# sriram-0311/MC-SLAM

Hardware: AMD Instinct MI355X
Metric: multi-cam frames/sec (4-cam 1280x720 @2000 kpts/cam, extract + intra-rig match) (higher is better)
Workload: dtype u8; 1 GPU; 4-cam rig 1280x720, 2000 kpts/cam, extract + all-pairs intra-rig match (configs[1]); slots=4, frames_per_launch=128, cameras=4, nfeatures=2000

## Files before the change

include/mcorb.h:

```cpp
#ifndef MCORB_H
#define MCORB_H

#include <stdint.h>
#include <stddef.h>

#ifdef __cplusplus
extern "C" {
#endif

#define MCORB_OK 0
#define MCORB_E_EMPTY (-1)
#define MCORB_E_SIZE (-2)
#define MCORB_E_CAP (-3)
#define MCORB_E_ARG (-4)
#define MCORB_E_HIP (-5)
#define MCORB_E_NODEVICE (-6)
#define MCORB_E_STATE (-7)
#define MCORB_E_OVERFLOW (-8)

#define MCORB_MAX_LEVELS 16
#define MCORB_MAX_CAMS 16
#define MCORB_SELECT_AUTO 0
#define MCORB_SELECT_HOST 1
#define MCORB_SELECT_GPU 2
// ... 10 lines not shown
    float scale_factor;
    int nlevels;
    int ini_th_fast;
    int min_th_fast;
    int orientation;
    int device_id;
    int host_threads;
    int cand_cap;
    int selection;
    int gpu_jobs;
    int reserved[5];
} mcorb_params;

void mcorb_default_params(mcorb_params *p);
const char *mcorb_last_error(void);
const char *mcorb_version(void);
int mcorb_device_count(void);

typedef struct mcorb_rig mcorb_rig;

int mcorb_rig_create(const mcorb_params *p, int ncams, int width, int height, int max_frames,
                     int nslots, mcorb_rig **out);
void mcorb_rig_destroy(mcorb_rig *r);

int mcorb_rig_upload_u8(mcorb_rig *r, int slot, const uint8_t *const *images, int nimg, int stride);
int mcorb_rig_staging(mcorb_rig *r, int slot, int m, uint8_t **ptr, int *stride);
int mcorb_rig_upload_staged(mcorb_rig *r, int slot, int nimg);
int mcorb_rig_upload_f32(mcorb_rig *r, int slot, const float *const *images, int nimg,
                         int stride_bytes, int channels);

int mcorb_rig_extract_submit(mcorb_rig *r, int slot, int nimg, int lap_x0, int lap_x1);
int mcorb_rig_extract_wait(mcorb_rig *r, int slot);
int mcorb_rig_extract(mcorb_rig *r, int slot, int nimg, int lap_x0, int lap_x1);

int mcorb_rig_process_submit(mcorb_rig *r, int slot, int nframes, int lap_x0, int lap_x1,
                             float dist_thresh, float ratio);
int mcorb_rig_process_wait(mcorb_rig *r, int slot);
int mcorb_rig_process(mcorb_rig *r, int slot, int nframes, int lap_x0, int lap_x1, float dist_thresh, float ratio);

int mcorb_rig_num_keypoints(mcorb_rig *r, int slot, int m);
int mcorb_rig_get_features(mcorb_rig *r, int slot, int m, mcorb_keypoint *kps, uint8_t *desc, int cap,
                           int *n_out, int *mono_index_out);

int mcorb_rig_set_undistortion(mcorb_rig *r, int cam, const double *K, const double *dist, int ncoeffs);
int mcorb_rig_undistortion_active(mcorb_rig *r, int cam);
int mcorb_rig_get_features_undist(mcorb_rig *r, int slot, int m, mcorb_keypoint *kps, int cap, int *n_out);

int mcorb_rig_set_image_undistortion(mcorb_rig *r, int cam, const double *K, const double *dist, int ncoeffs);
int mcorb_rig_image_undistortion_active(mcorb_rig *r, int cam);
int mcorb_rig_get_undistort_map(mcorb_rig *r, int cam, int16_t *map1_xy, uint16_t *map2, int cap_pixels);
int mcorb_rig_get_raw_image(mcorb_rig *r, int slot, int m, uint8_t *dst, int dst_stride);
int mcorb_host_undistort_map(const double *K, const double *dist, int ncoeffs, int w, int h, int16_t *map1_xy, uint16_t *map2);
int mcorb_host_remap_u8(const uint8_t *src, int src_stride, int w, int h, const int16_t *map1_xy, const uint16_t *map2,
                        uint8_t *dst, int dst_stride);

int mcorb_rig_match(mcorb_rig *r, int slot, int nframes, float dist_thresh, float ratio);
int mcorb_rig_match_submit(mcorb_rig *r, int slot, int nframes, float dist_thresh, float ratio);
int mcorb_rig_match_wait(mcorb_rig *r, int slot);
int mcorb_rig_get_pair_matches(mcorb_rig *r, int slot, int frame, int cam_i, int cam_j,
                               uint32_t *idx1, uint32_t *idx2, int cap, int *n_out);
int mcorb_rig_get_pair_knn2(mcorb_rig *r, int slot, int frame, int cam_i, int cam_j,
                            int32_t *idx, int32_t *dist, int cap_rows, int *nq_out);
int mcorb_rig_get_tracks(mcorb_rig *r, int slot, int frame, int32_t *tracks, int cap_tracks,
                         int *ntracks_out, int *mergeable_out);

int mcorb_rig_get_tracks_epipolar(mcorb_rig *r, int slot, int frame, const double *F, const mcorb_keypoint *const *kps_undist,
                                  int32_t *tracks, int cap_tracks, int *ntracks_out, int *mergeable_out);

int mcorb_rig_level_size(mcorb_rig *r, int level, int *w, int *h);
int mcorb_rig_get_level(mcorb_rig *r, int slot, int m, int level, uint8_t *dst, int dst_stride);
int mcorb_rig_get_blurred(mcorb_rig *r, int slot, int m, int level, uint8_t *dst, int dst_stride);
int mcorb_rig_get_candidates(mcorb_rig *r, int slot, int m, int level, uint32_t *packed, int cap, int *n_out);

int mcorb_rig_last_timing(mcorb_rig *r, int slot, float us[10]);
int mcorb_rig_select_mode(mcorb_rig *r);
int mcorb_rig_select_fallbacks(mcorb_rig *r, int slot);
int mcorb_rig_early_reads_rejected(mcorb_rig *r, int slot);
int mcorb_rig_set_graph(mcorb_rig *r, int every);
int mcorb_dev_sort_selftest(int device, const uint32_t *keys, int n, uint32_t *perm_dev, uint32_t *perm_std);

int mcorb_rig_kcap(mcorb_rig *r);
int mcorb_rig_host_threads(mcorb_rig *r);
int mcorb_rig_info(mcorb_rig *r, int32_t out[8]);
void *mcorb_rig_desc_device_ptr(mcorb_rig *r, int slot);
void *mcorb_rig_stream(mcorb_rig *r, int slot);
int mcorb_rig_export_descriptors(mcorb_rig *r, int slot, void *dst_dev, int32_t *counts_host, int nimg);
int mcorb_rig_match_external(mcorb_rig *r, int slot, const void *desc_dev, const int32_t *counts, int ntotal,
                             const int32_t *sets, int nframes, float dist_thresh, float ratio);
int mcorb_rig_match_external_submit(mcorb_rig *r, int slot, const void *desc_dev, const int32_t *counts, int ntotal,
                                    const int32_t *sets, int nframes, float dist_thresh, float ratio);

int mcorb_rig_export_descriptors_dev(mcorb_rig *r, int slot, void *dst_dev, int32_t *counts_dev, int nimg, void *then_stream);
int mcorb_rig_match_external_dev_submit(mcorb_rig *r, int slot, const void *desc_dev, const int32_t *counts_dev, int ntotal,
                                        const int32_t *sets, int nframes, float dist_thresh, float ratio, void *after_stream);

int mcorb_rig_match_pairs_external(mcorb_rig *r, int slot, const void *desc_dev, const int32_t *counts, int ntotal,
                                   const int32_t *pair_sets, int npairs, float dist_thresh, float ratio);
int mcorb_rig_match_pairs_external_dev_submit(mcorb_rig *r, int slot, const void *desc_dev, const int32_t *counts_dev, int ntotal,
                                              const int32_t *pair_sets, int npairs, float dist_thresh, float ratio, void *after_stream);
int mcorb_rig_get_pairlist(mcorb_rig *r, int slot, int pair, uint32_t *idx1, uint32_t *idx2, int cap, int *n_out);
int mcorb_host_merge_tracks(int ncams, const int32_t *counts, const uint32_t *const *idx1, const uint32_t *const *idx2,
                            const int32_t *npair, int32_t *tracks, int cap_tracks, int *ntracks_out, int *mergeable_out);

typedef struct mcorb_descblock mcorb_descblock;
int mcorb_descblock_create(int device, int nsets, int kcap, mcorb_descblock **out);
void mcorb_descblock_destroy(mcorb_descblock *b);
int mcorb_descblock_upload(mcorb_descblock *b, int set, const uint8_t *desc, int n);
void *mcorb_descblock_desc_ptr(mcorb_descblock *b);
int32_t *mcorb_descblock_counts_dev(mcorb_descblock *b);
int mcorb_rig_match_sets(mcorb_rig *r, int slot, mcorb_descblock *b, const int32_t *pair_sets, int npairs, float dist_thresh, float ratio);
int mcorb_rig_get_pairknn2(mcorb_rig *r, int slot, int pair, int32_t *idx, int32_t *dist, int cap_rows, int *nq_out);

typedef struct mcorb_extractor mcorb_t;

int mcorb_create(const mcorb_params *p, int max_width, int max_height, mcorb_t **out);
void mcorb_destroy(mcorb_t *e);
int mcorb_extract(mcorb_t *e, const uint8_t *gray, int w, int h, int stride_bytes,
                  int lap_x0, int lap_x1, mcorb_keypoint *kps, uint8_t *desc, int cap,
                  int *n_out, int *mono_index_out);
int mcorb_extract_f32(mcorb_t *e, const float *img01, int w, int h, int stride_bytes, int channels,
                      int lap_x0, int lap_x1, mcorb_keypoint *kps, uint8_t *desc, int cap,
                      int *n_out, int *mono_index_out);
int mcorb_get_tables(const mcorb_params *p, float *scale, float *inv_scale, float *sigma2,
                     float *inv_sigma2, int *features_per_level);
int mcorb_get_pyramid_level(mcorb_t *e, int level, uint8_t *dst, int dst_stride, int *w, int *h);

int mcorb_hamming256(const uint8_t a[32], const uint8_t b[32]);
int mcorb_representative_desc(const uint8_t *descs, int n);
int mcorb_knn2(mcorb_t *e, const uint8_t *q, int nq, const uint8_t *t, int nt, int32_t *idx, int32_t *dist);
int mcorb_match_ratio(mcorb_t *e, const uint8_t *q, int nq, const uint8_t *t, int nt,
                      float dist_thresh, float ratio, uint32_t *idx1, uint32_t *idx2, int cap, int *n_out);

typedef struct mcorb_vocab mcorb_vocab;
int mcorb_vocab_create(int k, int L, int scoring, int weighting, const int32_t *parent, const uint8_t *is_leaf,
                       const uint8_t *desc, const double *weight, int nnodes, int device, mcorb_vocab **out);
int mcorb_vocab_load_text(const char *path, int device, mcorb_vocab **out);
void mcorb_vocab_destroy(mcorb_vocab *v);
int mcorb_vocab_info(const mcorb_vocab *v, int *k, int *L, int *nnodes, int *nwords);
int mcorb_vocab_transform(mcorb_vocab *v, const uint8_t *desc, int n, int levelsup, uint32_t *bow_ids, double *bow_vals,
                          int bow_cap, int *nbow, uint32_t *fv_nodes, int32_t *fv_offsets, int fv_cap, int *nfv,
                          int32_t *fv_feats, int feat_cap);
int mcorb_rig_transform_image(mcorb_rig *r, int slot, int m, mcorb_vocab *v, int levelsup, uint32_t *bow_ids,
                              double *bow_vals, int bow_cap, int *nbow, uint32_t *fv_nodes, int32_t *fv_offsets,
                              int fv_cap, int *nfv, int32_t *fv_feats, int feat_cap);

int mcorb_rig_transform_images(mcorb_rig *r, int slot, int img0, int nimg, mcorb_vocab *v, int levelsup);
int mcorb_rig_get_transform(mcorb_rig *r, int slot, int m, uint32_t *bow_ids, double *bow_vals, int bow_cap, int *nbow,
                            uint32_t *fv_nodes, int32_t *fv_offsets, int fv_cap, int *nfv, int32_t *fv_feats, int feat_cap);
int mcorb_rig_match_bow(mcorb_rig *r, int slot, int frame, mcorb_vocab *v, int levelsup, double max_neighbor_ratio,
                        int32_t *tracks, int32_t *n_rays, int cap_tracks, int *ntracks_out, uint32_t *words,
                        int cap_words, int *nwords_out);
int mcorb_rig_match_bow_frames(mcorb_rig *r, int slot, int frame0, int nframes, mcorb_vocab *v, int levelsup,
                               double max_neighbor_ratio, const float *const *y_undist);
int mcorb_rig_get_bow_tracks(mcorb_rig *r, int slot, int frame, int32_t *tracks, int32_t *n_rays, int cap_tracks,
                             int *ntracks_out, uint32_t *words, int cap_words, int *nwords_out);

#define MCORB_BOW_TRANSFORM 1
#define MCORB_BOW_MATCH 2
#define MCORB_BOW_MAX_KCAP 4096
int mcorb_rig_set_vocabulary(mcorb_rig *r, mcorb_vocab *v, int levelsup, double max_neighbor_ratio, int flags);

typedef struct mcorb_camera {
    double K[9];
    double Rt[12];
} mcorb_camera;
typedef struct mcorb_lf_feature {
// ... 188 lines not shown
    int32_t *match_dist;
    double *match_pt;
    int32_t n_proj[MCORB_MAX_CAMS], n_match[MCORB_MAX_CAMS];
    int32_t n_candidates, reserved;
} mcorb_track_out;
int mcorb_lmap_track(mcorb_lmap *m, const mcorb_track_view *view, const mcorb_track_frame *frame, const int32_t *lids, int n_lids,
                     double max_d2, int max_hamming, mcorb_track_out *out);
int mcorb_lmap_track_rig_frame(mcorb_lmap *m, const mcorb_track_view *view, mcorb_rig *r, int slot, int frame, const int32_t *lids,
                               int n_lids, double max_d2, int max_hamming, mcorb_track_out *out);
int mcorb_lmap_last_track_timing(mcorb_lmap *m, float us[2]);
int mcorb_lmap_last_track_timing4(mcorb_lmap *m, float us[4]);
int mcorb_lmap_last_track_timing5(mcorb_lmap *m, float us[5]);
int mcorb_lmap_track_submit(mcorb_lmap *m, const mcorb_track_view *view, const mcorb_track_frame *frame, const int32_t *lids, int n_lids,
                            double max_d2, int max_hamming, int want_pts);
int mcorb_lmap_track_rig_frame_submit(mcorb_lmap *m, const mcorb_track_view *view, mcorb_rig *r, int slot, int frame, const int32_t *lids,
                                      int n_lids, double max_d2, int max_hamming, int want_pts);
int mcorb_lmap_track_wait(mcorb_lmap *m, mcorb_track_out *out);
#define MCORB_TRACK_MAX_FRAMES 32
int mcorb_lmap_track_rig_frames_submit(mcorb_lmap *m, const mcorb_track_view *views, mcorb_rig *r, int slot, const int32_t *frames, int nf,
                                       const int32_t *lids, const int32_t *lid_first , double max_d2, int max_hamming,
                                       int want_pts);
int mcorb_lmap_track_frames_wait(mcorb_lmap *m, mcorb_track_out *outs, int n_outs);
int mcorb_lmap_track_rig_frames(mcorb_lmap *m, const mcorb_track_view *views, mcorb_rig *r, int slot, const int32_t *frames, int nf,
                                const int32_t *lids, const int32_t *lid_first, double max_d2, int max_hamming, int want_pts,
                                mcorb_track_out *outs);

#define MCORB_POSE_LANES 256
#define MCORB_POSE_NO_OBS 0
#define MCORB_POSE_NO_STEP 1
#define MCORB_POSE_CONVERGED 2
#define MCORB_POSE_MAX_ITER 3
typedef struct mcorb_pose_params {
    double inv_sigma2[MCORB_MAX_LEVELS];
    int32_t nlevels, max_iterations;
} mcorb_pose_params;
typedef struct mcorb_pose_result {
    double R[9], t[3];
    double cost_initial, cost_final;
    int32_t status, iterations[2], n_inliers, n_obs, reserved;
} mcorb_pose_result;
int mcorb_lmap_refine_pose(mcorb_lmap *m, int n, const int32_t *cam, const float *uv, const int32_t *octave, const int32_t *lids,
                           const double *pts, int ncams, const mcorb_track_cam *cams, const double *R, const double *t,
                           const mcorb_pose_params *params, mcorb_pose_result *res, uint8_t *inlier);
int mcorb_lmap_last_pose_timing(mcorb_lmap *m, float us[1]);
int mcorb_lmap_set_track_refine(mcorb_lmap *m, const mcorb_pose_params *params);
int mcorb_lmap_last_track_pose(mcorb_lmap *m, int f, mcorb_pose_result *out, uint8_t *flags, int cap);
void mcorb_pose_of_view(const mcorb_track_view *view, double R[9], double t[3]);
int mcorb_pose_eval(int ncams, const mcorb_track_cam *cams, int n, const int32_t *cam, const float *uv, const double *pts, const double *R,
                    const double *t, double *r, double *J, double *w);

#define MCORB_SAC_MAX_ITERATIONS 1024
#define MCORB_SAC_SOLVER_CENTRAL 0
#define MCORB_SAC_SOLVER_RIG 1
#define MCORB_SAC_OK 0
#define MCORB_SAC_NO_OBS 1
#define MCORB_SAC_NO_MODEL 2
typedef struct mcorb_sac_params {
    double threshold;
    uint64_t seed;
    int32_t max_iterations, solver;
} mcorb_sac_params;
typedef struct mcorb_sac_result {
    double R[9], t[3];
    double sac_R[9], sac_t[3];
    int32_t status, used, n_inliers, n_matches;
    int32_t sac_n_inliers, best_hypothesis, sample[4], n_models, n_consensus;
    mcorb_pose_result refine;
} mcorb_sac_result;
int mcorb_lmap_ransac_pose(mcorb_lmap *m, int n, const int32_t *cam, const float *uv, const int32_t *octave, const int32_t *match,
                           const int32_t *lids, const double *pts, int ncams, const mcorb_track_cam *cams,
                           const mcorb_sac_params *params, const mcorb_pose_params *refine_params, mcorb_sac_result *res,
                           uint8_t *inlier);
int mcorb_lmap_last_ransac_timing(mcorb_lmap *m, float us[3], int *n_hyp);
int mcorb_lmap_last_ransac_counts(mcorb_lmap *m, int32_t *count, int32_t *valid, int cap, int *n_hyp);
double mcorb_sac_threshold(double K00_02);
int mcorb_sac_solve(const mcorb_track_cam *cam, const float *uv, const double *pts, double *R, double *t);
int mcorb_sac_solve_rig(int ncams, const mcorb_track_cam *cams, const int32_t *cam, const float *uv, const double *pts, double *R, double *t);
int mcorb_sac_eval(int ncams, const mcorb_track_cam *cams, int n, const int32_t *cam, const float *uv, const double *pts, const double *R,
                   const double *t, double *score);

int mcorb_host_select(const uint32_t *packed, int n, int minX, int maxX, int minY, int maxY,
                      int nfeatures_level, int wCell, int hCell, int32_t *out_idx, int cap);
int mcorb_host_resize_axis(int ssize, int dsize, int is_x, int32_t *quads);
int mcorb_host_geometry(const mcorb_params *p, int w, int h, int32_t *six_per_level);
int mcorb_host_triangulate(const double *x, const double *P, int nv, double X[3]);
int mcorb_host_triangulate_branch(const double *x, const double *P, int nv, double X[3], int32_t *branch);
int32_t mcorb_host_track_pixel(float v);

int mcorb_synth_rig_frame(uint32_t frame, int ncams, int cam, int w, int h, uint8_t *out, int stride);

#ifdef __cplusplus
}
#endif
#endif
```

mc-slam_amd/__init__.py:

```python
import ctypes as C

import numpy as np

from . import _lib
from ._lib import (E_ARG, E_CAP, E_EMPTY, E_HIP, E_NODEVICE, E_OVERFLOW, E_SIZE, E_STATE, KP_DTYPE, OBS_RECORD, OBS_UPDATE, OK,
                   ORIENT_IC_ANGLE, ORIENT_NONE, McorbError, Params, default_params)
from .synth import synth_rig_frame, synth_rig_frame_numpy

TH_HIGH = 100
TH_LOW = 75
HISTO_LENGTH = 30


def _u8(a):
    return np.ascontiguousarray(a, dtype=np.uint8)


def device_count():
    return _lib.load().mcorb_device_count()


def get_tables(params):
    n = params.nlevels
    sc, isc, s2, is2 = (np.zeros(n, np.float32) for _ in range(4))
    q = np.zeros(n, np.int32)
    _lib.check(_lib.load().mcorb_get_tables(C.byref(params), sc.ctypes.data, isc.ctypes.data, s2.ctypes.data,
                                            is2.ctypes.data, q.ctypes.data))
    return dict(scale=sc, inv_scale=isc, sigma2=s2, inv_sigma2=is2, quota=q)


def hamming256(a, b):
    a, b = _u8(a).reshape(32), _u8(b).reshape(32)
    return _lib.load().mcorb_hamming256(a.ctypes.data, b.ctypes.data)


def representative_desc(descs):
    d = _u8(descs).reshape(-1, 32)
    r = _lib.load().mcorb_representative_desc(d.ctypes.data, len(d))
    if r < 0:
        _lib.check(r)
    return r


class Rig:

    def __init__(self, ncams, width, height, max_frames=1, nslots=1, params=None, **kw):
        self.L = _lib.load()
        self.params = params if params is not None else default_params(**kw)
        self.ncams, self.w, self.h, self.max_frames, self.nslots = ncams, width, height, max_frames, nslots
        h = C.c_void_p()
        _lib.check(self.L.mcorb_rig_create(C.byref(self.params), ncams, width, height, max_frames, nslots, C.byref(h)))
        self.h_rig = h
        self.kcap = self.L.mcorb_rig_kcap(h)
        self.nlevels = self.params.nlevels

    def close(self):
        if getattr(self, "h_rig", None):
            self.L.mcorb_rig_destroy(self.h_rig)
            self.h_rig = None

    def __del__(self):
        try:
            self.close()
        except Exception:
            pass

    def upload(self, images, slot=0):
        first = np.asarray(images[0])
        if first.dtype == np.uint8:
            arrs = [_u8(im) for im in images]
            for a in arrs:
                if a.shape != (self.h, self.w):
                    raise ValueError("image shape %s != (%d,%d)" % (a.shape, self.h, self.w))
            ptrs = (C.c_void_p * len(arrs))(*[a.ctypes.data for a in arrs])
            _lib.check(self.L.mcorb_rig_upload_u8(self.h_rig, slot, ptrs, len(arrs), self.w))
        else:
            arrs = [np.ascontiguousarray(im, dtype=np.float32) for im in images]
            ch = 1 if arrs[0].ndim == 2 else arrs[0].shape[2]
            ptrs = (C.c_void_p * len(arrs))(*[a.ctypes.data for a in arrs])
            _lib.check(self.L.mcorb_rig_upload_f32(self.h_rig, slot, ptrs, len(arrs), arrs[0].strides[0], ch))
        return len(arrs)

    def staging(self, m, slot=0):
        ptr, stride = C.c_void_p(), C.c_int()
        _lib.check(self.L.mcorb_rig_staging(self.h_rig, slot, m, C.byref(ptr), C.byref(stride)))
        buf = (C.c_uint8 * (self.h * stride.value)).from_address(ptr.value)
        return np.frombuffer(buf, np.uint8).reshape(self.h, stride.value)[:, :self.w]

    def upload_staged(self, nimg, slot=0):
        _lib.check(self.L.mcorb_rig_upload_staged(self.h_rig, slot, nimg))

    def extract(self, nimg, slot=0, lap=(0, 0)):
        _lib.check(self.L.mcorb_rig_extract(self.h_rig, slot, nimg, lap[0], lap[1]))

# ... 176 lines not shown
            for c in range(Cn):
                a = np.ascontiguousarray(kps_undist[c], _lib.KP_DTYPE)
                keep.append(a)
                undp[c] = a.ctypes.data
        wp = None
        if words is not None:
            words = np.ascontiguousarray(words, np.uint32)
            assert len(words) >= len(tracks)
            wp = words.ctypes.data
        cap = max(total_feats, len(tracks)) + 1
        out = np.empty(cap, _lib.LF_DTYPE)
        wf = np.zeros(len(tracks) + 1, np.uint32)
        n, ni, nm, nw = (C.c_int() for _ in range(4))
        _lib.check(self.L.mcorb_rig_obtain_lf_features(self.h_rig, slot, frame, tracks.ctypes.data, len(tracks), wp, cams, segp, stride, undp,
                                                       total_feats, out.ctypes.data, cap, C.byref(n), C.byref(ni), C.byref(nm),
                                                       wf.ctypes.data, len(wf), C.byref(nw)))
        return out[:n.value].copy(), ni.value, nm.value, wf[:nw.value].copy()

    def obtain_lf_features_frames(self, frame0, tracks_per_frame, K_mats, R_mats, t_mats, words_per_frame=None, seg_masks=None,
                                  kps_undist=None, total_feats=3000, slot=0):
        Cn, F = self.ncams, len(tracks_per_frame)
        trs = [np.ascontiguousarray(t, np.int32).reshape(-1, Cn) for t in tracks_per_frame]
        nt = np.array([len(t) for t in trs], np.int32)
        tracks = np.ascontiguousarray(np.concatenate(trs) if nt.sum() else np.zeros((0, Cn), np.int32))
        cams = (_lib.Camera * Cn)()
        for c in range(Cn):
            K = np.asarray(K_mats[c], np.float64).reshape(3, 3)
            Rt = np.hstack([np.asarray(R_mats[c], np.float64).reshape(3, 3), np.asarray(t_mats[c], np.float64).reshape(3, 1)])
            cams[c].K[:] = K.ravel().tolist()
            cams[c].Rt[:] = Rt.ravel().tolist()
        keep, segp, stride = [], None, 0
        if seg_masks is not None:
            segp = (C.c_void_p * (F * Cn))()
            for i in range(F * Cn):
                if seg_masks[i] is not None:
                    a = np.ascontiguousarray(seg_masks[i], np.float32)
                    assert stride in (0, a.shape[1]), "all segmentation masks must share one row stride"
                    keep.append(a)
                    segp[i] = a.ctypes.data
                    stride = a.shape[1]
        undp = None
        if kps_undist is not None:
            undp = (C.c_void_p * (F * Cn))()
            for i in range(F * Cn):
                a = np.ascontiguousarray(kps_undist[i], _lib.KP_DTYPE)
                keep.append(a)
                undp[i] = a.ctypes.data
        wp = None
        if words_per_frame is not None:
            ws = [np.ascontiguousarray(w, np.uint32)[:n] for w, n in zip(words_per_frame, nt)]
            assert all(len(w) == n for w, n in zip(ws, nt)), "one word per track"
            words = np.ascontiguousarray(np.concatenate(ws) if nt.sum() else np.zeros(0, np.uint32))
            keep.append(words)
            wp = words.ctypes.data
        cap = max(total_feats, int(nt.max(initial=0))) + 1
        capw = int(nt.max(initial=0)) + 1
        out = np.empty((F, cap), _lib.LF_DTYPE)
        wf = np.zeros((F, capw), np.uint32)
        n, ni, nm, nw = (np.zeros(F, np.int32) for _ in range(4))
        _lib.check(self.L.mcorb_rig_obtain_lf_features_frames(self.h_rig, slot, frame0, F, tracks.ctypes.data, nt.ctypes.data, wp, cams, segp,
                                                              stride, undp, total_feats, out.ctypes.data, cap, n.ctypes.data, ni.ctypes.data,
                                                              nm.ctypes.data, wf.ctypes.data, capw, nw.ctypes.data))
        return [(out[f, :n[f]].copy(), int(ni[f]), int(nm[f]), wf[f, :nw[f]].copy()) for f in range(F)]

    def level_size(self, level):
        w, h = C.c_int(), C.c_int()
        _lib.check(self.L.mcorb_rig_level_size(self.h_rig, level, C.byref(w), C.byref(h)))
        return w.value, h.value

    def level(self, m, level, slot=0, blurred=False):
        w, h = self.level_size(level)
        out = np.zeros((h, w), np.uint8)
        fn = self.L.mcorb_rig_get_blurred if blurred else self.L.mcorb_rig_get_level
        _lib.check(fn(self.h_rig, slot, m, level, out.ctypes.data, w))
        return out

    def candidates(self, m, level, slot=0, cap=1 << 17):
        buf = np.zeros(cap, np.uint32)
        n = C.c_int()
        _lib.check(self.L.mcorb_rig_get_candidates(self.h_rig, slot, m, level, buf.ctypes.data, cap, C.byref(n)))
        p = buf[:n.value]
        return ((p >> 8) & 0xfff).astype(np.int32), (p >> 20).astype(np.int32), (p & 0xff).astype(np.int32)

    def info(self):
        o = np.zeros(8, np.int32)
        _lib.check(self.L.mcorb_rig_info(self.h_rig, o.ctypes.data))
        d = dict(zip(("kcap", "cells", "tiles", "cell_cap", "cand_cap", "bucket_total", "img_bytes", "nlevels"), (int(v) for v in o)))
        d["host_threads"] = int(self.L.mcorb_rig_host_threads(self.h_rig))
        return d

    def select_mode(self):
        return {1: "host", 2: "gpu"}[self.L.mcorb_rig_select_mode(self.h_rig)]

    def set_graph(self, every):
        _lib.check(self.L.mcorb_rig_set_graph(self.h_rig, every))

    def select_fallbacks(self, slot=0):
        return int(self.L.mcorb_rig_select_fallbacks(self.h_rig, slot))

    def early_reads_rejected(self, slot=0):
        return int(self.L.mcorb_rig_early_reads_rejected(self.h_rig, slot))

    def timing(self, slot=0):
        t = (C.c_float * 10)()
        _lib.check(self.L.mcorb_rig_last_timing(self.h_rig, slot, t))
        return dict(phase_a_us=t[0], select_us=t[1], phase_b_us=t[2], match_us=t[3], pyramid_us=t[4],
                    fast_us=t[5], compact_us=t[6], knn2_us=t[7], blur_us=t[8], describe_us=t[9])

    def export_descriptors(self, dst_dev_ptr, nimg, slot=0):
        counts = np.zeros(nimg, np.int32)
        _lib.check(self.L.mcorb_rig_export_descriptors(self.h_rig, slot, dst_dev_ptr, counts.ctypes.data, nimg))
        return counts

    def match_external(self, desc_dev_ptr, counts, sets, slot=0, dist_thresh=75.0, ratio=0.85):
        self.match_external_submit(desc_dev_ptr, counts, sets, slot, dist_thresh, ratio)
        self.match_wait(slot)

    def match_external_submit(self, desc_dev_ptr, counts, sets, slot=0, dist_thresh=75.0, ratio=0.85):
        counts = np.ascontiguousarray(counts, np.int32)
        sets = np.ascontiguousarray(sets, np.int32).reshape(-1, self.ncams)
        self._keep = getattr(self, "_keep", {})
        self._keep[slot] = (counts, sets)
        _lib.check(self.L.mcorb_rig_match_external_submit(self.h_rig, slot, desc_dev_ptr, counts.ctypes.data, len(counts),
                                                          sets.ctypes.data, len(sets), dist_thresh, ratio))

    def export_descriptors_dev(self, dst_dev_ptr, counts_dev_ptr, nimg, slot=0, then_stream=None):
        if then_stream:
            _lib.require_torch_first("export_descriptors_dev")
        _lib.check(self.L.mcorb_rig_export_descriptors_dev(self.h_rig, slot, dst_dev_ptr, counts_dev_ptr, nimg, then_stream))

    def match_external_dev_submit(self, desc_dev_ptr, counts_dev_ptr, ntotal, sets, slot=0, dist_thresh=75.0, ratio=0.85,
                                  after_stream=None):
        if after_stream:
            _lib.require_torch_first("match_external_dev_submit")
        sets = np.ascontiguousarray(sets, np.int32).reshape(-1, self.ncams)
        self._keep = getattr(self, "_keep", {})
        self._keep[slot] = (sets,)
        _lib.check(self.L.mcorb_rig_match_external_dev_submit(self.h_rig, slot, desc_dev_ptr, counts_dev_ptr, int(ntotal),
                                                              sets.ctypes.data, len(sets), dist_thresh, ratio, after_stream))

    def match_wait(self, slot=0):
        _lib.check(self.L.mcorb_rig_match_wait(self.h_rig, slot))

    def match_pairs_external(self, desc_dev_ptr, counts, pair_sets, slot=0, dist_thresh=75.0, ratio=0.85):
        counts = np.ascontiguousarray(counts, np.int32)
        pair_sets = np.ascontiguousarray(pair_sets, np.int32).reshape(-1, 2)
        _lib.check(self.L.mcorb_rig_match_pairs_external(self.h_rig, slot, desc_dev_ptr, counts.ctypes.data, len(counts),
                                                         pair_sets.ctypes.data, len(pair_sets), dist_thresh, ratio))

    def match_pairs_external_dev_submit(self, desc_dev_ptr, counts_dev_ptr, ntotal, pair_sets, slot=0, dist_thresh=75.0, ratio=0.85,
                                        after_stream=None):
        if after_stream:
            _lib.require_torch_first("match_pairs_external_dev_submit")
        pair_sets = np.ascontiguousarray(pair_sets, np.int32).reshape(-1, 2)
        self._keep = getattr(self, "_keep", {})
        self._keep[slot] = (pair_sets,)
        _lib.check(self.L.mcorb_rig_match_pairs_external_dev_submit(self.h_rig, slot, desc_dev_ptr, counts_dev_ptr, int(ntotal),
                                                                    pair_sets.ctypes.data, len(pair_sets), dist_thresh, ratio, after_stream))

    def match_sets(self, block, pair_sets, slot=0, dist_thresh=75.0, ratio=0.85):
        pair_sets = np.ascontiguousarray(pair_sets, np.int32).reshape(-1, 2)
        _lib.check(self.L.mcorb_rig_match_sets(self.h_rig, slot, block.h, pair_sets.ctypes.data, len(pair_sets), dist_thresh, ratio))

    def pairknn2(self, pair, slot=0):
        idx, dist = np.zeros((self.kcap, 2), np.int32), np.zeros((self.kcap, 2), np.int32)
        n = C.c_int()
        _lib.check(self.L.mcorb_rig_get_pairknn2(self.h_rig, slot, pair, idx.ctypes.data, dist.ctypes.data, self.kcap, C.byref(n)))
        return idx[:n.value].copy(), dist[:n.value].copy()

    def pairlist(self, pair, slot=0):
        i1, i2 = np.zeros(self.kcap, np.uint32), np.zeros(self.kcap, np.uint32)
        n = C.c_int()
# ... 1309 lines not shown
```

mc-slam_amd/_lib.py:

```python
import ctypes as C
import os
import sys

import numpy as np

PKG_DIR = os.path.dirname(os.path.abspath(__file__))
LIB_PATH = os.path.join(PKG_DIR, "libmcorb.so")

OK, E_EMPTY, E_SIZE, E_CAP, E_ARG, E_HIP, E_NODEVICE, E_STATE, E_OVERFLOW = 0, -1, -2, -3, -4, -5, -6, -7, -8
ORIENT_NONE, ORIENT_IC_ANGLE = 0, 1
BOW_TRANSFORM, BOW_MATCH = 1, 2
OBS_UPDATE, OBS_RECORD = 0, 1
MAX_LEVELS, MAX_CAMS = 16, 16
TRACK_KNN, TRACK_TILE = 10, 1024
TRACK_MAX_FRAMES = 32
POSE_LANES = 256
POSE_NO_OBS, POSE_NO_STEP, POSE_CONVERGED, POSE_MAX_ITER = 0, 1, 2, 3

KP_DTYPE = np.dtype([("x", "<f4"), ("y", "<f4"), ("size", "<f4"), ("angle", "<f4"),
                     ("response", "<f4"), ("octave", "<i4"), ("class_id", "<i4")])


class Params(C.Structure):
    _fields_ = [("nfeatures", C.c_int), ("scale_factor", C.c_float), ("nlevels", C.c_int),
# ... 76 lines not shown
    _fields_ = [("R", C.c_double * 9), ("t", C.c_double * 3), ("cost_initial", C.c_double), ("cost_final", C.c_double),
                ("status", C.c_int32), ("iterations", C.c_int32 * 2), ("n_inliers", C.c_int32), ("n_obs", C.c_int32),
                ("reserved", C.c_int32)]


class SacParams(C.Structure):
    _fields_ = [("threshold", C.c_double), ("seed", C.c_uint64), ("max_iterations", C.c_int32), ("solver", C.c_int32)]


class SacResultC(C.Structure):
    _fields_ = [("R", C.c_double * 9), ("t", C.c_double * 3), ("sac_R", C.c_double * 9), ("sac_t", C.c_double * 3),
                ("status", C.c_int32), ("used", C.c_int32), ("n_inliers", C.c_int32), ("n_matches", C.c_int32),
                ("sac_n_inliers", C.c_int32), ("best_hypothesis", C.c_int32), ("sample", C.c_int32 * 4), ("n_models", C.c_int32),
                ("n_consensus", C.c_int32), ("refine", PoseResultC)]


class McorbError(RuntimeError):
    def __init__(self, code, msg):
        super().__init__("mcorb error %d: %s" % (code, msg))
        self.code = code


_vp, _i, _f = C.c_void_p, C.c_int, C.c_float
_ip = C.POINTER(C.c_int)

SIGNATURES = {
    "mcorb_default_params": (None, [C.POINTER(Params)]),
    "mcorb_last_error": (C.c_char_p, []),
    "mcorb_version": (C.c_char_p, []),
    "mcorb_device_count": (_i, []),
    "mcorb_rig_create": (_i, [C.POINTER(Params), _i, _i, _i, _i, _i, C.POINTER(_vp)]),
    "mcorb_rig_destroy": (None, [_vp]),
    "mcorb_rig_upload_u8": (_i, [_vp, _i, C.POINTER(_vp), _i, _i]),
    "mcorb_rig_upload_f32": (_i, [_vp, _i, C.POINTER(_vp), _i, _i, _i]),
    "mcorb_rig_extract_submit": (_i, [_vp, _i, _i, _i, _i]),
    "mcorb_rig_extract_wait": (_i, [_vp, _i]),
    "mcorb_rig_extract": (_i, [_vp, _i, _i, _i, _i]),
    "mcorb_rig_staging": (_i, [_vp, _i, _i, _vp, _ip]),
    "mcorb_rig_upload_staged": (_i, [_vp, _i, _i]),
    "mcorb_rig_process_submit": (_i, [_vp, _i, _i, _i, _i, _f, _f]),
    "mcorb_rig_process": (_i, [_vp, _i, _i, _i, _i, _f, _f]),
    "mcorb_rig_process_wait": (_i, [_vp, _i]),
    "mcorb_rig_num_keypoints": (_i, [_vp, _i, _i]),
    "mcorb_rig_get_features": (_i, [_vp, _i, _i, _vp, _vp, _i, _ip, _ip]),
    "mcorb_rig_set_undistortion": (_i, [_vp, _i, _vp, _vp, _i]),
    "mcorb_rig_undistortion_active": (_i, [_vp, _i]),
    "mcorb_rig_get_features_undist": (_i, [_vp, _i, _i, _vp, _i, _ip]),
    "mcorb_rig_set_image_undistortion": (_i, [_vp, _i, _vp, _vp, _i]),
    "mcorb_rig_image_undistortion_active": (_i, [_vp, _i]),
    "mcorb_rig_get_undistort_map": (_i, [_vp, _i, _vp, _vp, _i]),
    "mcorb_rig_get_raw_image": (_i, [_vp, _i, _i, _vp, _i]),
    "mcorb_host_undistort_map": (_i, [_vp, _vp, _i, _i, _i, _vp, _vp]),
    "mcorb_host_remap_u8": (_i, [_vp, _i, _i, _i, _vp, _vp, _vp, _i]),
    "mcorb_rig_match": (_i, [_vp, _i, _i, _f, _f]),
    "mcorb_rig_match_submit": (_i, [_vp, _i, _i, _f, _f]),
    "mcorb_rig_match_wait": (_i, [_vp, _i]),
    "mcorb_rig_get_pair_matches": (_i, [_vp, _i, _i, _i, _i, _vp, _vp, _i, _ip]),
    "mcorb_rig_get_pair_knn2": (_i, [_vp, _i, _i, _i, _i, _vp, _vp, _i, _ip]),
    "mcorb_rig_get_tracks": (_i, [_vp, _i, _i, _vp, _i, _ip, _ip]),
    "mcorb_rig_level_size": (_i, [_vp, _i, _ip, _ip]),
    "mcorb_rig_get_level": (_i, [_vp, _i, _i, _i, _vp, _i]),
    "mcorb_rig_get_blurred": (_i, [_vp, _i, _i, _i, _vp, _i]),
    "mcorb_rig_get_candidates": (_i, [_vp, _i, _i, _i, _vp, _i, _ip]),
    "mcorb_rig_last_timing": (_i, [_vp, _i, C.POINTER(_f)]),
    "mcorb_rig_select_mode": (_i, [_vp]),
    "mcorb_rig_select_fallbacks": (_i, [_vp, _i]),
    "mcorb_rig_early_reads_rejected": (_i, [_vp, _i]),
    "mcorb_rig_set_graph": (_i, [_vp, _i]),
    "mcorb_dev_sort_selftest": (_i, [_i, _vp, _i, _vp, _vp]),
    "mcorb_rig_match_pairs_external": (_i, [_vp, _i, _vp, _vp, _i, _vp, _i, _f, _f]),
    "mcorb_rig_match_pairs_external_dev_submit": (_i, [_vp, _i, _vp, _vp, _i, _vp, _i, _f, _f, _vp]),
    "mcorb_rig_get_pairlist": (_i, [_vp, _i, _i, _vp, _vp, _i, _ip]),
    "mcorb_host_merge_tracks": (_i, [_i, _vp, _vp, _vp, _vp, _vp, _i, _ip, _ip]),
    "mcorb_descblock_create": (_i, [_i, _i, _i, _vp]),
    "mcorb_descblock_destroy": (None, [_vp]),
    "mcorb_descblock_upload": (_i, [_vp, _i, _vp, _i]),
    "mcorb_descblock_desc_ptr": (_vp, [_vp]),
    "mcorb_descblock_counts_dev": (_vp, [_vp]),
    "mcorb_rig_match_sets": (_i, [_vp, _i, _vp, _vp, _i, _f, _f]),
    "mcorb_rig_get_pairknn2": (_i, [_vp, _i, _i, _vp, _vp, _i, _ip]),
    "mcorb_rig_kcap": (_i, [_vp]),
    "mcorb_rig_host_threads": (_i, [_vp]),
    "mcorb_rig_info": (_i, [_vp, _vp]),
    "mcorb_rig_desc_device_ptr": (_vp, [_vp, _i]),
    "mcorb_rig_stream": (_vp, [_vp, _i]),
    "mcorb_rig_export_descriptors": (_i, [_vp, _i, _vp, _vp, _i]),
    "mcorb_rig_match_external": (_i, [_vp, _i, _vp, _vp, _i, _vp, _i, _f, _f]),
    "mcorb_rig_match_external_submit": (_i, [_vp, _i, _vp, _vp, _i, _vp, _i, _f, _f]),
    "mcorb_rig_export_descriptors_dev": (_i, [_vp, _i, _vp, _vp, _i, _vp]),
    "mcorb_rig_match_external_dev_submit": (_i, [_vp, _i, _vp, _vp, _i, _vp, _i, _f, _f, _vp]),
    "mcorb_create": (_i, [C.POINTER(Params), _i, _i, C.POINTER(_vp)]),
    "mcorb_destroy": (None, [_vp]),
    "mcorb_extract": (_i, [_vp, _vp, _i, _i, _i, _i, _i, _vp, _vp, _i, _ip, _ip]),
    "mcorb_extract_f32": (_i, [_vp, _vp, _i, _i, _i, _i, _i, _i, _vp, _vp, _i, _ip, _ip]),
    "mcorb_get_tables": (_i, [C.POINTER(Params), _vp, _vp, _vp, _vp, _vp]),
    "mcorb_get_pyramid_level": (_i, [_vp, _i, _vp, _i, _ip, _ip]),
    "mcorb_hamming256": (_i, [_vp, _vp]),
    "mcorb_representative_desc": (_i, [_vp, _i]),
    "mcorb_knn2": (_i, [_vp, _vp, _i, _vp, _i, _vp, _vp]),
    "mcorb_match_ratio": (_i, [_vp, _vp, _i, _vp, _i, _f, _f, _vp, _vp, _i, _ip]),
    "mcorb_vocab_create": (_i, [_i, _i, _i, _i, _vp, _vp, _vp, _vp, _i, _i, C.POINTER(_vp)]),
    "mcorb_vocab_load_text": (_i, [C.c_char_p, _i, C.POINTER(_vp)]),
    "mcorb_vocab_destroy": (None, [_vp]),
    "mcorb_vocab_info": (_i, [_vp, _ip, _ip, _ip, _ip]),
    "mcorb_vocab_transform": (_i, [_vp, _vp, _i, _i, _vp, _vp, _i, _ip, _vp, _vp, _i, _ip, _vp, _i]),
    "mcorb_rig_transform_image": (_i, [_vp, _i, _i, _vp, _i, _vp, _vp, _i, _ip, _vp, _vp, _i, _ip, _vp, _i]),
    "mcorb_rig_get_tracks_epipolar": (_i, [_vp, _i, _i, _vp, _vp, _vp, _i, _ip, _ip]),
    "mcorb_rig_match_bow": (_i, [_vp, _i, _i, _vp, _i, C.c_double, _vp, _vp, _i, _ip, _vp, _i, _ip]),
    "mcorb_rig_transform_images": (_i, [_vp, _i, _i, _i, _vp, _i]),
    "mcorb_rig_get_transform": (_i, [_vp, _i, _i, _vp, _vp, _i, _ip, _vp, _vp, _i, _ip, _vp, _i]),
    "mcorb_rig_match_bow_frames": (_i, [_vp, _i, _i, _i, _vp, _i, C.c_double, _vp]),
    "mcorb_rig_set_vocabulary": (_i, [_vp, _vp, _i, C.c_double, _i]),
    "mcorb_rig_get_bow_tracks": (_i, [_vp, _i, _i, _vp, _vp, _i, _ip, _vp, _i, _ip]),
    "mcorb_rig_obtain_lf_features": (_i, [_vp, _i, _i, _vp, _i, _vp, _vp, _vp, _i, _vp, _i, _vp, _i, _ip, _ip, _ip, _vp, _i, _ip]),
    "mcorb_rig_obtain_lf_features_frames": (_i, [_vp, _i, _i, _i, _vp, _vp, _vp, _vp, _vp, _i, _vp, _i, _vp, _i, _vp, _vp, _vp, _vp, _i, _vp]),
    "mcorb_host_select": (_i, [_vp, _i, _i, _i, _i, _i, _i, _i, _i, _vp, _i]),
    "mcorb_host_resize_axis": (_i, [_i, _i, _i, _vp]),
    "mcorb_host_triangulate": (_i, [_vp, _vp, _i, _vp]),
    "mcorb_host_triangulate_branch": (_i, [_vp, _vp, _i, _vp, _vp]),
    "mcorb_rig_set_lf": (_i, [_vp, _vp, _i]),
    "mcorb_rig_get_lf_features": (_i, [_vp, _i, _i, _vp, _i, _ip, _ip, _ip, _vp, _i, _ip]),
    "mcorb_rig_get_lf_bow": (_i, [_vp, _i, _i, _vp, _vp, _i, _ip, _vp, _vp, _i, _ip, _vp, _i]),
    "mcorb_dev_triangulate_selftest": (_i, [_i, _vp, _vp, _vp, _i, _vp, _vp]),
    "mcorb_kfdb_create": (_i, [_vp, _i, _i, _i, _i, C.POINTER(_vp)]),
    "mcorb_kfdb_destroy": (None, [_vp]),
    "mcorb_kfdb_add": (_i, [_vp, _vp, _vp, _i, _vp, _vp, _i, _vp, _vp, _i, _ip]),
    "mcorb_kfdb_add_rig_frame": (_i, [_vp, _vp, _i, _i, _ip]),
    "mcorb_kfdb_size": (_i, [_vp]),
    "mcorb_kfdb_get_entry": (_i, [_vp, _i, _vp, _vp, _i, _ip, _vp, _vp, _i, _ip, _vp, _i, _vp, _i, _ip]),
    "mcorb_kfdb_query": (_i, [_vp, _vp, _vp, _i, _i, _i, _vp, _vp, _i, _ip]),
    "mcorb_kfdb_query_entries": (_i, [_vp, _vp, _vp, _i, _i, _vp, _vp, _i, _vp]),
    "mcorb_kfdb_score": (_i, [_vp, _i, _i, C.POINTER(C.c_double)]),
    "mcorb_kfdb_feature_matches": (_i, [_vp, _i, _i, C.c_double, _vp, _vp, _i, _ip]),
    "mcorb_kfdb_last_timing": (_i, [_vp, C.POINTER(_f)]),
    "mcorb_kfdb_reserve_probes": (_i, [_vp, _i]),
    "mcorb_kfdb_set_probe": (_i, [_vp, _i, _vp, _vp, _i, _vp, _vp, _i, _vp, _vp, _i]),
    "mcorb_kfdb_set_probe_rig_frame": (_i, [_vp, _i, _vp, _i, _i]),
    "mcorb_kfdb_get_probe": (_i, [_vp, _i, _vp, _vp, _i, _ip, _vp, _vp, _i, _ip, _vp, _i, _vp, _i, _ip]),
    "mcorb_kfdb_query_probes": (_i, [_vp, _vp, _vp, _i, _i, _vp, _vp, _i, _vp]),
    "mcorb_kfdb_score_probe": (_i, [_vp, _i, _i, C.POINTER(C.c_double)]),
    "mcorb_kfdb_probe_feature_matches": (_i, [_vp, _i, _vp, _i, C.c_double, _vp, _vp, _i, _vp]),
    "mcorb_kfdb_probe_inter_matches_bf": (_i, [_vp, _i, _i, _vp, _vp, _vp, _vp, _vp, _vp, _vp, _vp, _i, _ip]),
    "mcorb_kfdb_last_probe_timing": (_i, [_vp, C.POINTER(_f)]),
    "mcorb_lmap_create": (_i, [_vp, _i, _i, _i, C.POINTER(_vp)]),
    "mcorb_lmap_destroy": (None, [_vp]),
    "mcorb_lmap_set": (_i, [_vp, _vp, _i, _vp, _vp, _vp, _vp]),
    "mcorb_lmap_set_desc_from_entry": (_i, [_vp, _vp, _i, _vp, _vp, _i, _vp]),
    "mcorb_lmap_get": (_i, [_vp, _i, _vp, _vp, _vp, _ip, _ip]),
    "mcorb_lmap_search": (_i, [_vp, C.POINTER(LmapView), _vp, _i, _vp, _i, _vp, _i, _vp, _vp, _vp, _i, C.c_double, _vp, _vp, _i, _ip,
                               _vp, _vp, _i, _ip, _vp, _vp, _i, _ip]),
    "mcorb_lmap_last_timing": (_i, [_vp, C.POINTER(_f), _ip]),
    "mcorb_lmap_triangulate_neighbours": (_i, [_vp, C.POINTER(MapFrame), _vp, C.POINTER(MapFrame), C.POINTER(_vp), _i, C.POINTER(_vp),
                                               C.POINTER(_vp), C.POINTER(_vp), _vp, _vp, _vp, _i, _vp, _vp, C.c_int32,
                                               C.POINTER(MapOut)]),
    "mcorb_lmap_depths": (_i, [_vp, _vp, _vp, _vp, _i, _vp]),
    "mcorb_lmap_last_triangulate_timing": (_i, [_vp, C.POINTER(_f), _ip, _ip]),
    "mcorb_lmap_triangulate_new": (_i, [_vp, C.POINTER(MapFrame), _vp, C.POINTER(MapFrame), _vp, _vp, _vp, _i, _vp, _vp, _i, _i,
                                        C.POINTER(MapNewOut)]),
    "mcorb_lmap_last_triangulate_new_timing": (_i, [_vp, C.POINTER(_f), _ip]),
    "mcorb_host_map_refine": (_i, [_i] + [_vp] * 11 + [_i] + [_vp] * 5),
    "mcorb_dev_map_refine_selftest": (_i, [_i, _i] + [_vp] * 11 + [_i] + [_vp] * 5),
    "mcorb_host_map_gates": (_i, [_i, _vp, _vp, _vp, _vp, _vp, _vp, _vp, _vp, _vp, _vp, _i, _vp, _vp, _vp]),
    "mcorb_dev_map_gates_selftest": (_i, [_i, _i, _vp, _vp, _vp, _vp, _vp, _vp, _vp, _vp, _vp, _vp, _i, _vp, _vp, _vp]),
    "mcorb_lmap_set_rays": (_i, [_vp, _vp, _i, _vp]),
    "mcorb_lmap_get_observations": (_i, [_vp, _i, C.POINTER(C.c_int32), _vp, _vp, _i, _ip]),
    "mcorb_lmap_observe": (_i, [_vp, C.POINTER(ObsFrame), _vp, _vp, _i, _i, _vp, _i, _vp, _vp]),
    "mcorb_lmap_update_points": (_i, [_vp, _vp, _i, _vp, C.c_double, _vp, _vp]),
    "mcorb_lmap_delete": (_i, [_vp, _vp, _i, _vp, _vp, _i, _ip]),
    "mcorb_lmap_observers": (_i, [_vp, _vp, _i, _vp, _i, _ip]),
    "mcorb_lmap_last_landmark_timing": (_i, [_vp, C.POINTER(_f)]),
    "mcorb_lmap_track": (_i, [_vp, C.POINTER(TrackView), C.POINTER(TrackFrame), _vp, _i, C.c_double, _i, C.POINTER(TrackOut)]),
    "mcorb_lmap_track_rig_frame": (_i, [_vp, C.POINTER(TrackView), _vp, _i, _i, _vp, _i, C.c_double, _i, C.POINTER(TrackOut)]),
    "mcorb_lmap_last_track_timing": (_i, [_vp, C.POINTER(_f)]),
    "mcorb_lmap_last_track_timing4": (_i, [_vp, C.POINTER(_f)]),
    "mcorb_lmap_last_track_timing5": (_i, [_vp, C.POINTER(_f)]),
    "mcorb_lmap_track_submit": (_i, [_vp, C.POINTER(TrackView), C.POINTER(TrackFrame), _vp, _i, C.c_double, _i, _i]),
    "mcorb_lmap_track_rig_frame_submit": (_i, [_vp, C.POINTER(TrackView), _vp, _i, _i, _vp, _i, C.c_double, _i, _i]),
    "mcorb_lmap_track_wait": (_i, [_vp, C.POINTER(TrackOut)]),
    "mcorb_lmap_track_rig_frames_submit": (_i, [_vp, C.POINTER(TrackView), _vp, _i, _vp, _i, _vp, _vp, C.c_double, _i, _i]),
    "mcorb_lmap_track_frames_wait": (_i, [_vp, C.POINTER(TrackOut), _i]),
    "mcorb_lmap_track_rig_frames": (_i, [_vp, C.POINTER(TrackView), _vp, _i, _vp, _i, _vp, _vp, C.c_double, _i, _i, C.POINTER(TrackOut)]),
    "mcorb_host_track_pixel": (C.c_int32, [_f]),
    "mcorb_lmap_refine_pose": (_i, [_vp, _i, _vp, _vp, _vp, _vp, _vp, _i, _vp, _vp, _vp, C.POINTER(PoseParams), C.POINTER(PoseResultC), _vp]),
    "mcorb_lmap_last_pose_timing": (_i, [_vp, C.POINTER(_f)]),
    "mcorb_lmap_set_track_refine": (_i, [_vp, C.POINTER(PoseParams)]),
    "mcorb_lmap_last_track_pose": (_i, [_vp, _i, C.POINTER(PoseResultC), _vp, _i]),
    "mcorb_pose_of_view": (None, [C.POINTER(TrackView), _vp, _vp]),
    "mcorb_pose_eval": (_i, [_i, _vp, _i, _vp, _vp, _vp, _vp, _vp, _vp, _vp, _vp]),
    "mcorb_lmap_ransac_pose": (_i, [_vp, _i, _vp, _vp, _vp, _vp, _vp, _vp, _i, _vp, C.POINTER(SacParams), C.POINTER(PoseParams),
                                    C.POINTER(SacResultC), _vp]),
    "mcorb_lmap_last_ransac_timing": (_i, [_vp, C.POINTER(_f), C.POINTER(_i)]),
    "mcorb_lmap_last_ransac_counts": (_i, [_vp, _vp, _vp, _i, C.POINTER(_i)]),
    "mcorb_sac_threshold": (C.c_double, [C.c_double]),
    "mcorb_sac_solve": (_i, [_vp, _vp, _vp, _vp, _vp]),
    "mcorb_sac_solve_rig": (_i, [_i, _vp, _vp, _vp, _vp, _vp, _vp]),
    "mcorb_sac_eval": (_i, [_i, _vp, _i, _vp, _vp, _vp, _vp, _vp, _vp]),
    "mcorb_host_geometry": (_i, [C.POINTER(Params), _i, _i, _vp]),
    "mcorb_synth_rig_frame": (_i, [C.c_uint32, _i, _i, _i, _i, _vp, _i]),
}

# ... 41 lines not shown
```

mc-slam_amd/csrc/mcorb_api.cpp:

```cpp
#include <string.h>

#include <algorithm>
#include <cmath>
#include <chrono>
#include <new>

#include "mcorb_engine.h"

using namespace mcorb;

extern "C" {

void mcorb_default_params(mcorb_params *p)
{
    if (!p) return;
    memset(p, 0, sizeof(*p));
    p->nfeatures = 2000;
    p->scale_factor = 1.2f;
    p->nlevels = 8;
    p->ini_th_fast = 20;
    p->min_th_fast = 7;
    p->orientation = MCORB_ORIENT_NONE;
}

// ... 369 lines not shown
    Slot *s = get_slot(r, slot);
    if (!s) return MCORB_E_STATE;
    const Geom &g = r->rig.geom;
    if (m < 0 || m >= s->nimg_done || level < 0 || level >= g.nlevels) { set_error("bad candidate request"); return MCORB_E_ARG; }
    int dev_lo[kMaxLevels + 1];
    const int *lo = s->tbl(m) + kTblLvlOff;
    if (!(s->host_results && !r->rig.gpu_select)) {
        HIPCHK(hipSetDevice(r->rig.device));
        HIPCHK(hipMemcpy(dev_lo, s->d_tbl + (size_t)m * s->tbl_ints_per_image + kTblLvlOff, sizeof(dev_lo), hipMemcpyDeviceToHost));
        lo = dev_lo;
    }
    const int n = lo[level + 1] - lo[level];
    if (n_out) *n_out = n;
    if (n > cap) { set_error("candidate buffer too small"); return MCORB_E_CAP; }
    if (n) {
        std::vector<uint32_t> tmp(n);
        HIPCHK(hipSetDevice(r->rig.device));
        HIPCHK(hipMemcpy(tmp.data(), s->d_sorted + (size_t)m * g.candCap + lo[level], (size_t)n * 4, hipMemcpyDeviceToHost));
        const uint32_t *src = tmp.data();
        const int wc = g.lv[level].wCell, hc = g.lv[level].hCell;
        std::vector<std::pair<uint64_t, uint32_t>> v(n);
        for (int i = 0; i < n; i++) {
            const int x = cand_x(src[i]), y = cand_y(src[i]);
            v[i] = {((((uint64_t)((y - 3) / hc) << 12 | (uint64_t)((x - 3) / wc)) << 12 | (uint64_t)y) << 12) | (uint64_t)x, src[i]};
        }
        std::sort(v.begin(), v.end());
        for (int i = 0; i < n; i++) packed[i] = v[i].second;
    }
    return MCORB_OK;
}

int mcorb_rig_last_timing(mcorb_rig *r, int slot, float us[10])
{
    Slot *s = get_slot(r, slot);
    if (!s) return MCORB_E_STATE;
    for (int i = 0; i < T_COUNT; i++) us[i] = s->timing[i];
    return MCORB_OK;
}

int mcorb_rig_kcap(mcorb_rig *r) { return r ? r->rig.geom.kcap : MCORB_E_ARG; }
int mcorb_rig_select_mode(mcorb_rig *r) { return r ? (r->rig.gpu_select ? MCORB_SELECT_GPU : MCORB_SELECT_HOST) : MCORB_E_ARG; }
int mcorb_rig_set_graph(mcorb_rig *r, int every)
{
    if (!r || every < 0) return MCORB_E_ARG;
    r->rig.graph_every.store(r->rig.gpu_select ? every : 0);
    return MCORB_OK;
}
int mcorb_rig_select_fallbacks(mcorb_rig *r, int slot)
{
    if (!r || slot < 0 || slot >= (int)r->rig.slots.size()) return MCORB_E_ARG;
    return r->rig.slots[slot]->fallbacks.load(std::memory_order_relaxed);
}
int mcorb_rig_early_reads_rejected(mcorb_rig *r, int slot)
{
    if (!r || slot < 0 || slot >= (int)r->rig.slots.size()) return MCORB_E_ARG;
    return r->rig.slots[slot]->stale_reads.load(std::memory_order_relaxed);
}
int mcorb_dev_sort_selftest(int device, const uint32_t *keys, int n, uint32_t *dev_perm, uint32_t *std_perm)
{
    if (n < 0 || n > 6000 || (n && (!keys || !dev_perm || !std_perm))) { set_error("sort_selftest: bad argument"); return MCORB_E_ARG; }
    if (n == 0) return MCORB_OK;
    std::vector<uint64_t> a((size_t)n), b((size_t)n);
    for (int i = 0; i < n; i++) a[i] = ((uint64_t)keys[i] << 32) | (uint32_t)i;
    b = a;
    std::sort(b.begin(), b.end(), [](uint64_t x, uint64_t y) { return (x >> 32) < (y >> 32); });
    for (int i = 0; i < n; i++) std_perm[i] = (uint32_t)b[i];
    HIPCHK(hipSetDevice(device));
    DevBuf<uint64_t> d_in, d_out;
    TRY(d_in.alloc((size_t)n));
    TRY(d_out.alloc((size_t)n));
    HIPCHK(hipMemcpy(d_in, a.data(), (size_t)n * 8, hipMemcpyHostToDevice));
    HIPCHK(sort_selftest(d_in, n, d_out));
    HIPCHK(hipMemcpy(b.data(), d_out, (size_t)n * 8, hipMemcpyDeviceToHost));
    for (int i = 0; i < n; i++) dev_perm[i] = (uint32_t)b[i];
    return MCORB_OK;
}
int mcorb_rig_host_threads(mcorb_rig *r) { return r ? r->rig.pool_threads : MCORB_E_ARG; }
int mcorb_rig_info(mcorb_rig *r, int32_t out[8])
{
    if (!r || !out) return MCORB_E_ARG;
    const Geom &g = r->rig.geom;
    out[0] = g.kcap; out[1] = g.cells; out[2] = g.tiles; out[3] = g.cellCap; out[4] = g.candCap; out[5] = g.bucketTotal;
    out[6] = (int32_t)g.imgBytes; out[7] = g.nlevels;
    return MCORB_OK;
}
void *mcorb_rig_desc_device_ptr(mcorb_rig *r, int slot)
{
    if (!r || slot < 0 || slot >= (int)r->rig.slots.size()) return nullptr;
    return r->rig.slots[slot]->d_desc;
}
void *mcorb_rig_stream(mcorb_rig *r, int slot)
{
    if (!r || slot < 0 || slot >= (int)r->rig.slots.size()) return nullptr;
    return (void *)r->rig.slots[slot]->st;
}

int mcorb_rig_match_external_submit(mcorb_rig *r, int slot, const void *desc_dev, const int32_t *counts, int ntotal,
                                    const int32_t *sets, int nframes, float dist_thresh, float ratio)
{
    if (!r || !desc_dev || !counts || !sets) { set_error("null argument"); return MCORB_E_ARG; }
    Job j = match_job(nframes, dist_thresh, ratio);
    j.ext_desc = desc_dev; j.ext_counts = counts; j.ext_total = ntotal; j.ext_sets = sets;
    return r->rig.submit(slot, j);
}

int mcorb_rig_match_external(mcorb_rig *r, int slot, const void *desc_dev, const int32_t *counts, int ntotal,
                             const int32_t *sets, int nframes, float dist_thresh, float ratio)
{
    const int st = mcorb_rig_match_external_submit(r, slot, desc_dev, counts, ntotal, sets, nframes, dist_thresh, ratio);
    return st != MCORB_OK ? st : r->rig.wait(slot);
}

int mcorb_rig_match_external_dev_submit(mcorb_rig *r, int slot, const void *desc_dev, const int32_t *counts_dev, int ntotal,
                                        const int32_t *sets, int nframes, float dist_thresh, float ratio, void *after_stream)
{
    if (!r || !desc_dev || !counts_dev || !sets) { set_error("null argument"); return MCORB_E_ARG; }
    Job j = match_job(nframes, dist_thresh, ratio);
    j.ext_desc = desc_dev; j.ext_counts_dev = counts_dev; j.ext_total = ntotal; j.ext_sets = sets;
    j.after_stream = (hipStream_t)after_stream;
    if (after_stream) {
        Slot *s = get_slot(r, slot);
        if (!s) return MCORB_E_STATE;
        HIPCHK(hipSetDevice(r->rig.device));
        HIPCHK(hipEventRecord(s->ev_x, (hipStream_t)after_stream));
    }
    return r->rig.submit(slot, j);
}

int mcorb_rig_match_pairs_external_dev_submit(mcorb_rig *r, int slot, const void *desc_dev, const int32_t *counts_dev, int ntotal,
                                              const int32_t *pair_sets, int npairs, float dist_thresh, float ratio, void *after_stream)
{
    if (!r || !desc_dev || !counts_dev || !pair_sets) { set_error("null argument"); return MCORB_E_ARG; }
    Job j = match_job(0, dist_thresh, ratio);
    j.ext_desc = desc_dev; j.ext_counts_dev = counts_dev; j.ext_total = ntotal; j.ext_pairs = pair_sets; j.ext_npairs = npairs;
    j.after_stream = (hipStream_t)after_stream;
    if (after_stream) {
        Slot *s = get_slot(r, slot);
        if (!s) return MCORB_E_STATE;
        HIPCHK(hipSetDevice(r->rig.device));
        HIPCHK(hipEventRecord(s->ev_x, (hipStream_t)after_stream));
    }
    return r->rig.submit(slot, j);
}

int mcorb_rig_match_pairs_external(mcorb_rig *r, int slot, const void *desc_dev, const int32_t *counts, int ntotal,
                                   const int32_t *pair_sets, int npairs, float dist_thresh, float ratio)
{
    if (!r || !desc_dev || !counts || !pair_sets) { set_error("null argument"); return MCORB_E_ARG; }
    Job j = match_job(0, dist_thresh, ratio);
    j.ext_desc = desc_dev; j.ext_counts = counts; j.ext_total = ntotal; j.ext_pairs = pair_sets; j.ext_npairs = npairs;
    return r->rig.run_sync(slot, j);
}

int mcorb_rig_get_pairlist(mcorb_rig *r, int slot, int pair, uint32_t *idx1, uint32_t *idx2, int cap, int *n_out)
{
    if (n_out) *n_out = 0;
    Slot *s = get_slot(r, slot);
    if (!s) return MCORB_E_STATE;
    if (pair < 0 || pair >= s->npairs_done) { set_error("bad pair index"); return MCORB_E_ARG; }
    const int n = (int)s->m_idx1[pair].size();
    if (n_out) *n_out = n;
    if (n > cap || (n && (!idx1 || !idx2))) { set_error("pair list: output too small"); return MCORB_E_CAP; }
    if (n) {
        memcpy(idx1, s->m_idx1[pair].data(), (size_t)n * sizeof(uint32_t));
        memcpy(idx2, s->m_idx2[pair].data(), (size_t)n * sizeof(uint32_t));
    }
// ... 130 lines not shown
```

mc-slam_amd/csrc/mcorb_api_extractor.cpp:

```cpp
#include <string.h>

#include <algorithm>
#include <new>

#include "mcorb_engine.h"

using namespace mcorb;

struct mcorb_extractor {
    mcorb_params params;
    std::unique_ptr<Rig> rig;
    int w = 0, h = 0;
    DevBuf<uint8_t> d_desc, d_exp;
    DevBuf<int> d_lcounts;
    DevBuf<uint2> d_part;
    HostBuf<KnnRow> h_rows;
    HostBuf<uint32_t> h_mlist;
    HostBuf<int> h_mcount, h_counts;
    HostBuf<int2> h_pair;
    int kc = 0;
};

extern "C" {

// ... 166 lines not shown
        TRY(e->d_lcounts.alloc(2));
        TRY(e->h_rows.alloc((size_t)need, hipHostMallocMapped));
        TRY(e->h_mlist.alloc(knn_mlist_stride(need), hipHostMallocMapped));
        TRY(e->h_mcount.alloc((size_t)knn_qblocks(need), hipHostMallocMapped));
        TRY(e->h_counts.alloc(2, hipHostMallocMapped));
        TRY(e->h_pair.alloc(1, hipHostMallocMapped));
        e->kc = need;
    }
    if (nq) HIPCHK(hipMemcpy(e->d_desc, q, (size_t)nq * 32, hipMemcpyHostToDevice));
    if (nt) HIPCHK(hipMemcpy(e->d_desc + (size_t)e->kc * 32, t, (size_t)nt * 32, hipMemcpyHostToDevice));
    e->h_counts[0] = nq;
    e->h_counts[1] = nt;
    e->h_pair[0] = int2{0, 1};
    launch_knn2(nullptr, e->d_desc, e->h_counts, nullptr, 2, e->h_pair, 1, e->kc, e->d_exp, e->d_lcounts, e->d_part, thr, ratio, e->h_rows,
                e->h_mlist, e->h_mcount, nullptr, nullptr);
    HIPCHK(hipGetLastError());
    HIPCHK(hipStreamSynchronize(nullptr));
    return MCORB_OK;
}

int mcorb_knn2(mcorb_t *e, const uint8_t *q, int nq, const uint8_t *t, int nt, int32_t *idx, int32_t *dist)
{
    if (!idx || !dist) { set_error("null output"); return MCORB_E_ARG; }
    const int st = knn2_host_arrays(e, q, nq, t, nt, 75.f, 0.85f);
    if (st != MCORB_OK) return st;
    decode_rows(e->h_rows, nq, idx, dist);
    return MCORB_OK;
}

int mcorb_match_ratio(mcorb_t *e, const uint8_t *q, int nq, const uint8_t *t, int nt, float dist_thresh, float ratio,
                      uint32_t *idx1, uint32_t *idx2, int cap, int *n_out)
{
    const int st = knn2_host_arrays(e, q, nq, t, nt, dist_thresh, ratio);
    if (st != MCORB_OK) return st;
    int n = 0;
    for (int i = 0; i < nq; i++) {
        const KnnRow &r = e->h_rows[i];
        if (knn_accept(r)) {
            if (n < cap) { idx1[n] = (uint32_t)i; idx2[n] = (uint32_t)knn_idx0(r); }
            n++;
        }
    }
    if (n_out) *n_out = n;
    if (n > cap) { set_error("match buffer too small"); return MCORB_E_CAP; }
    return MCORB_OK;
}

int mcorb_host_select(const uint32_t *packed, int n, int minX, int maxX, int minY, int maxY, int nfeatures_level,
                      int wCell, int hCell, int32_t *out_idx, int cap)
{
    if (n < 0 || (n && !packed) || !out_idx) { set_error("host_select: bad argument"); return MCORB_E_ARG; }
    if (n == 0) return 0;
    const SelectParams P = make_select_params(minX, maxX, minY, maxY, nfeatures_level, wCell, hCell);
    if (P.nIni < 1) { set_error("host_select: level too tall"); return MCORB_E_SIZE; }
    static thread_local SelectScratch sc;
    std::vector<uint32_t> sorted;
    std::vector<int> perm, bstart;
    std::vector<mcorb::BucketBest> bbest;
    host_bucket_sort(packed, n, P, sorted, perm, bstart, bbest);
    std::vector<int> out((size_t)std::max(nfeatures_level, 0) + 64 + 8);
    std::vector<uint32_t> outv(out.size());
    const int r = select_octree(sorted.data(), bstart.data(), bbest.data(), n, P, out.data(), outv.data(), sc);
    if (r == -4) { set_error("host_select: 2^20 candidates or a level 4096 px wide: beyond the packed (count, UL.x) sort key"); return MCORB_E_SIZE; }
    if (r < 0) { set_error("host_select: level too tall"); return MCORB_E_SIZE; }
    if (r > cap) { set_error("host_select: output too small"); return MCORB_E_CAP; }
    for (int i = 0; i < r; i++) {
        out_idx[i] = perm[out[i]];
        if (outv[i] != packed[out_idx[i]]) { set_error("host_select: value/index mismatch"); return MCORB_E_STATE; }
    }
    return r;
}

int mcorb_host_resize_axis(int ssize, int dsize, int is_x, int32_t *quads)
{
    if (ssize < 1 || dsize < 1 || !quads) return MCORB_E_ARG;
    std::vector<ResizeTap> t;
    build_resize_axis(ssize, dsize, is_x != 0, t, 1);
    for (int d = 0; d < dsize; d++) {
        quads[4 * d] = t[d].s0; quads[4 * d + 1] = t[d].s1; quads[4 * d + 2] = t[d].c0; quads[4 * d + 3] = t[d].c1;
    }
    return MCORB_OK;
}

int mcorb_host_geometry(const mcorb_params *p, int w, int h, int32_t *six)
{
    if (!p || !six) return MCORB_E_ARG;
    Tables t;
    int st = compute_tables(*p, t);
    if (st != MCORB_OK) return st;
    Geom g;
    std::vector<ResizeTap> taps;
    st = build_geometry(*p, t, w, h, g, taps);
    if (st != MCORB_OK) return st;
    for (int l = 0; l < g.nlevels; l++) {
        const LevelGeom &L = g.lv[l];
        int32_t *o = six + 6 * l;
        o[0] = L.w; o[1] = L.h; o[2] = L.nCols; o[3] = L.nRows; o[4] = L.wCell; o[5] = L.hCell;
    }
    return MCORB_OK;
}

}
```

mc-slam_amd/csrc/mcorb_common.h:

```cpp
#pragma once
#include <stdint.h>
#include <stddef.h>

namespace mcorb {

constexpr int kMaxLevels = 16;
constexpr int kEdge = 19;
constexpr int kMinBorder = 16;
constexpr int kCellW = 35;
constexpr int kMaxRoi = 76;
constexpr int kResizeTileH = 32;
constexpr int kBlurTW = 128, kBlurTH = 32;
constexpr int kTilePitch = 80;

__host__ __device__ inline uint32_t pack_cand(int x, int y, int resp) { return ((uint32_t)y << 20) | ((uint32_t)x << 8) | (uint32_t)resp; }
__host__ __device__ inline int cand_x(uint32_t p) { return (int)((p >> 8) & 0xfffu); }
__host__ __device__ inline int cand_y(uint32_t p) { return (int)(p >> 20); }
__host__ __device__ inline int cand_resp(uint32_t p) { return (int)(p & 0xffu); }

constexpr int kPickOrderMask = (1 << 23) - 1;
struct BucketBest { uint32_t key, pos, val; };
struct BucketWin { uint32_t key, val; };

constexpr int kTblLvlOff = 0, kTblShipped = kMaxLevels + 1, kTblHead = 48;
// ... 34 lines not shown
__host__ __device__ inline void unpack_sel(uint32_t v, int &level, int &x, int &y)
{
    level = (int)(v >> 28);
    y = (int)((v >> 14) & 0x3fffu);
    x = (int)(v & 0x3fffu);
}

constexpr int kBlurTileRows = 8, kBlurTileCols = 16, kBlurTileBytes = 128;
#if defined(__HIPCC__)
__host__ __device__
#endif
inline size_t blur_tiled_offset(int pitch, int x, int y)
{
    return ((size_t)(y >> 3) * (size_t)(pitch >> 4) + (size_t)(x >> 4)) * kBlurTileBytes + (size_t)((y & 7) << 4) + (size_t)(x & 15);
}

struct LevelGeom {
    int w, h;
    int pitch;
    uint32_t off;
    int nCols, nRows;
    int wCell, hCell;
    int cell0;
    int tile0;
    int tilesX, tilesY;
    int maxBorderX, maxBorderY;
    uint32_t xtab, ytab;
    int nIni;
    float hX;
    int depth;
    int nBuckets;
    int bucket0;
    int quota;
    uint32_t lutx, luty;
};

struct Geom {
    int nlevels;
    int cells;
    int tiles;
    int cellCap;
    uint32_t imgBytes;
    int kcap;
    int candCap;
    int hostCandCap;
    int bucketTotal;
    LevelGeom lv[kMaxLevels];
};

__host__ __device__ inline uint32_t path_code(int x, int y, int W0, int H0, int nIni, float hX, int depth)
{
#if defined(__HIP_DEVICE_COMPILE__)
    int r = (int)__fdiv_rn((float)x, hX);
    if (r >= nIni) r = nIni - 1;
    int x0 = (int)__fmul_rn(hX, (float)r), x1 = (int)__fmul_rn(hX, (float)(r + 1));
#else
    int r = (int)((float)x / hX);
    if (r >= nIni) r = nIni - 1;
    int x0 = (int)(hX * (float)r), x1 = (int)(hX * (float)(r + 1));
#endif
    int y0 = 0, y1 = H0;
    (void)W0;
    uint32_t code = (uint32_t)r;
    for (int d = 0; d < depth; d++) {
        const int sx = x0 + ((x1 - x0 + 1) >> 1), sy = y0 + ((y1 - y0 + 1) >> 1);
        const int qx = x >= sx, qy = y >= sy;
        if (qx) x0 = sx; else x1 = sx;
        if (qy) y0 = sy; else y1 = sy;
        code = (code << 2) | (uint32_t)(qx + 2 * qy);
    }
    return code;
}

inline void path_code_tables(int W0, int H0, int nIni, float hX, int depth, uint16_t *tx, uint16_t *ty)
{
    uint32_t ymask = 0;
    for (int d = 0; d < depth; d++) ymask |= 2u << (2 * d);
    for (int x = 0; x < W0; x++) tx[x] = (uint16_t)(path_code(x, 0, W0, H0, nIni, hX, depth) & ~ymask);
    for (int y = 0; y < H0; y++) ty[y] = (uint16_t)(path_code(0, y, W0, H0, nIni, hX, depth) & ymask);
}

struct ResizeTap { uint16_t s0, s1; int16_t c0, c1; };

}
```

mc-slam_amd/csrc/mcorb_engine.cpp:

```cpp
#include <stdlib.h>
#include <string.h>
#include <sys/prctl.h>
#include <time.h>

#include "mcorb_engine.h"
#include "mcorb_prof.h"

namespace mcorb {

static thread_local std::string g_err;
void set_error(const std::string &msg) { g_err = msg; }
const char *get_error() { return g_err.c_str(); }
hipError_t Rig::wait_event(hipEvent_t ev) const
{
    if (wait_mode != 2) return hipEventSynchronize(ev);
    for (int i = 0;; i++) {
        const hipError_t e = hipEventQuery(ev);
        if (e != hipErrorNotReady) return e;
        if (i < 4) { std::this_thread::yield(); continue; }
        timespec ts = {0, 20000};
        nanosleep(&ts, nullptr);
    }
}

template <typename T>
static int host_alloc(HostBuf<T> &b, size_t n)
{
    TRY(b.alloc(n, kHostMapped));
    memset(b, 0, n * sizeof(T));
    return MCORB_OK;
}

int Rig::init(const mcorb_params &p, int ncams_, int W_, int H_, int max_frames_, int nslots)
{
    if (ncams_ < 1 || ncams_ > MCORB_MAX_CAMS || max_frames_ < 1 || nslots < 1 || W_ < 1 || H_ < 1) {
        set_error("bad rig arguments");
        return MCORB_E_ARG;
    }
    int ndev = 0;
    if (hipGetDeviceCount(&ndev) != hipSuccess || ndev <= 0 || p.device_id < 0 || p.device_id >= ndev) {
        set_error("no usable HIP device (libmcorb has no CPU path)");
        return MCORB_E_NODEVICE;
    }
    hipDeviceProp_t prop;
    HIPCHK(hipGetDeviceProperties(&prop, p.device_id));
    if (strncmp(prop.gcnArchName, "gfx950", 6) != 0) {
        set_error(std::string("device is ") + prop.gcnArchName + ", libmcorb is built for gfx950 only");
        return MCORB_E_NODEVICE;
    }
    params = p;
    ncams = ncams_; W = W_; H = H_; max_frames = max_frames_;
    max_images = ncams * max_frames;
    undist_cams.assign(ncams, UndistCam{});
    undist_set.assign(ncams, 0);
    imgud_cams.assign(ncams, UndistImageCam{});
    imgud_set.assign(ncams, 0);
    imgud_map1.assign(ncams, {});
    imgud_map2.assign(ncams, {});
    d_imgud_map1.resize(ncams);
    d_imgud_map2.resize(ncams);
    npp = ncams * (ncams - 1) / 2;
    device = p.device_id;
    HIPCHK(hipSetDevice(device));
    TRY(compute_tables(p, tab));
    std::vector<ResizeTap> taps;
    std::vector<uint16_t> lut;
    TRY(build_geometry(p, tab, W, H, geom, taps, &lut));
    for (int l = 0; l < geom.nlevels; l++)
        selp[l] = make_select_params(kMinBorder, geom.lv[l].maxBorderX, kMinBorder, geom.lv[l].maxBorderY, tab.quota[l],
                                     geom.lv[l].wCell, geom.lv[l].hCell);
    if (taps.empty()) taps.push_back(ResizeTap{0, 0, 0, 0});
    TRY(resize_windows(geom, taps, resize_win));
    TRY(d_taps.alloc(taps.size()));
    HIPCHK(hipMemcpy(d_taps, taps.data(), taps.size() * sizeof(ResizeTap), hipMemcpyHostToDevice));
    TRY(d_lut.alloc(lut.size() + 8));
    HIPCHK(hipMemcpy(d_lut, lut.data(), lut.size() * sizeof(uint16_t), hipMemcpyHostToDevice));
    {
        std::vector<uint32_t> ft;
        fast_cell_off = fast_cell_table(geom, ft);
        TRY(d_fasttab.alloc(ft.size()));
        HIPCHK(hipMemcpy(d_fasttab, ft.data(), ft.size() * sizeof(uint32_t), hipMemcpyHostToDevice));
    }
    HIPCHK(upload_umax(tab.umax));

    const int cores = usable_cores();
    const char *sync_env = getenv("MCORB_SYNC");
    wait_mode = nslots > 1 ? 2 : 0;
    if (sync_env) wait_mode = !strcmp(sync_env, "block") ? 1 : (!strcmp(sync_env, "poll") ? 2 : 0);
    const bool blocking = wait_mode == 1;
    int nthreads = p.host_threads > 0 ? p.host_threads : (wait_mode == 0 ? cores - nslots - 2 : cores - 4);
    if (p.host_threads <= 0) nthreads = std::max(2, std::min(nthreads, std::min(max_images, 16)));
    if (getenv("MCORB_HOST_THREADS")) nthreads = atoi(getenv("MCORB_HOST_THREADS"));
    nthreads = std::max(1, std::min(nthreads, 64));
    blur_planes = p.orientation != 0 || getenv("MCORB_BLUR_PLANES") != nullptr;
    copy_kernel = getenv("MCORB_COPY_KERNEL") ? atoi(getenv("MCORB_COPY_KERNEL")) != 0 : nslots == 1;
    {
        const char *e = getenv("MCORB_SELECT");
        int mode = p.selection;
        if (mode == MCORB_SELECT_AUTO && e) mode = !strcmp(e, "host") ? MCORB_SELECT_HOST : (!strcmp(e, "gpu") ? MCORB_SELECT_GPU : MCORB_SELECT_AUTO);
        if (mode != MCORB_SELECT_AUTO && mode != MCORB_SELECT_HOST && mode != MCORB_SELECT_GPU) { set_error("mcorb_params.selection: unknown mode"); return MCORB_E_ARG; }
        gpu_select = mode != MCORB_SELECT_HOST && select_fits(geom);
        if (gpu_select) HIPCHK(configure_select(geom));
        if (getenv("MCORB_SELECT_DEEP_CAP")) select_deep_cap = std::max(1, atoi(getenv("MCORB_SELECT_DEEP_CAP")));
        compact_one_copy = getenv("MCORB_COMPACT_ONE_COPY") != nullptr;
        select_prof = getenv("MCORB_SELECT_PROF") != nullptr;
        gpu_job_limit = getenv("MCORB_GPU_JOBS") ? atoi(getenv("MCORB_GPU_JOBS")) : p.gpu_jobs;
        if (gpu_job_limit < 0 || gpu_job_limit >= nslots) gpu_job_limit = 0;
        upload_pipelined = !(getenv("MCORB_UPLOAD_PIPE") && atoi(getenv("MCORB_UPLOAD_PIPE")) == 0);
        graph_every = !gpu_select ? 0 : getenv("MCORB_GRAPH") ? std::max(0, atoi(getenv("MCORB_GRAPH"))) : (nslots == 1 ? 1 : 0);
    }
    pool.reset(new WorkerPool(nthreads));
    pool_threads = nthreads;
    for (int i = 0; i < nthreads + nslots; i++) scratch.emplace_back(new SelectScratch);

    const int npairs_max = std::max(1, npp * max_frames);
    ext_cap = (int)align_up(std::max((size_t)4096, (size_t)64 * max_images), 64);
    for (int si = 0; si < nslots; si++) {
        slots.emplace_back(new Slot);
        Slot *s = slots.back().get();
        s->rig = this;
        s->index = si;
        for (Stream *st : {&s->st, &s->st_copy, &s->st_dma}) TRY(st->create(hipStreamNonBlocking));
        TRY(s->ev_x.create(hipEventDisableTiming));
        for (Event *e : {&s->ev_c, &s->ev_e, &s->ev_start, &s->ev_pyr, &s->ev_fast, &s->ev_blur, &s->ev_desc0, &s->ev_desc1, &s->ev_knn0, &s->ev_knn1, &s->ev_fin})
            TRY(e->create(hipEventDefault));
        for (Event *e : {&s->ev_tables, &s->ev_done, &s->ev_side}) TRY(e->create(blocking ? hipEventBlockingSync : hipEventDefault));
        const size_t M = (size_t)max_images;
        TRY(s->d_pyr.alloc(M * geom.imgBytes));
        HIPCHK(hipMemset(s->d_pyr, 0, M * geom.imgBytes));
        if (blur_planes) {
            TRY(s->d_blur.alloc(M * geom.imgBytes));
            HIPCHK(hipMemset(s->d_blur, 0, M * geom.imgBytes));
        }
        TRY(s->d_cellkp.alloc(M * geom.cells * geom.cellCap));
        TRY(s->d_cellcnt.alloc(M * geom.cells));
        TRY(s->d_sorted.alloc(M * geom.candCap));
        s->tbl_ints_per_image = tbl_ints(geom.bucketTotal);
        TRY(s->d_tbl.alloc(M * s->tbl_ints_per_image));
        TRY(host_alloc(s->h_tbl, M * s->tbl_ints_per_image));
        TRY(s->d_desc.alloc(M * geom.kcap * 32));
        HIPCHK(hipMemset(s->d_desc, 0, M * geom.kcap * 32));
        TRY(s->d_angles.alloc(M * geom.kcap));
        TRY(s->d_part.alloc(knn_part_entries(npairs_max, geom.kcap)));
        TRY(s->d_exp.alloc(M * geom.kcap * (size_t)kKnnExpandBytes));
        TRY(s->d_lcounts.alloc(M));
        TRY(host_alloc(s->h_cand, M * geom.hostCandCap));
        TRY(host_alloc(s->h_overflow, 16));
        TRY(s->d_knn.alloc((size_t)npairs_max * geom.kcap));
        TRY(host_alloc(s->h_mlist, (size_t)npairs_max * knn_mlist_stride(geom.kcap)));
        TRY(host_alloc(s->h_mcount, (size_t)npairs_max * knn_qblocks(geom.kcap)));
        {
            const size_t o_nsel = (size_t)ext_cap * sizeof(int);
            const size_t o_setmap = align_up(o_nsel + M * sizeof(int), 64);
            const size_t o_pairs = align_up(o_setmap + M * sizeof(int), 64);
            const size_t o_sel = align_up(o_pairs + (size_t)npairs_max * sizeof(int2), 64);
// ... 118 lines not shown
        st = enqueue_match(s, j, false);
        if (st == MCORB_OK) {
            hipError_t e = hipEventRecord(s.ev_done, s.st);
            if (e == hipSuccess) e = wait_event(s.ev_done);
            if (e != hipSuccess) { set_error(hipGetErrorString(e)); st = MCORB_E_HIP; }
        }
        if (st == MCORB_OK) st = finish_match(s, j);
        break;
    default: break;
    }
    return st;
}

int Rig::run_sync(int slot, const Job &job)
{
    if (slot < 0 || slot >= (int)slots.size()) { set_error("bad slot"); return MCORB_E_ARG; }
    Slot &s = *slots[slot];
    TRY(check_job_shape(job));
    {
        std::lock_guard<std::mutex> lk(s.m);
        if (s.busy) { set_error("slot busy"); return MCORB_E_STATE; }
        s.busy = true;
        s.inline_job = true;
        s.status = MCORB_OK;
    }
    (void)hipSetDevice(device);
    const int st = execute(s, job);
    {
        std::lock_guard<std::mutex> lk(s.m);
        s.status = st;
        if (st != MCORB_OK) s.err = get_error();
        s.busy = false;
        s.inline_job = false;
    }
    s.cv.notify_all();
    return st;
}

void Rig::driver(Slot *sp)
{
    Slot &s = *sp;
    (void)hipSetDevice(device);
    if (wait_mode == 2) (void)prctl(PR_SET_TIMERSLACK, 2000UL, 0, 0, 0);
    for (;;) {
        Job j;
        {
            std::unique_lock<std::mutex> lk(s.m);
            s.cv.wait(lk, [&s] { return s.quit || (s.busy && !s.inline_job); });
            if (s.quit) return;
            j = s.job;
        }
        const int st = execute(s, j);
        {
            std::lock_guard<std::mutex> lk(s.m);
            s.status = st;
            if (st != MCORB_OK) s.err = get_error();
            s.busy = false;
        }
        s.cv.notify_all();
    }
}

int Rig::begin_extract(Slot &s, const Job &j)
{
    if (j.nimg < 1 || j.nimg > max_images) { set_error("extract: bad image count"); return MCORB_E_ARG; }
    s.invalidate_bow();
    s.bow_job = bow_bind.flags;
    s.lf_job = lf_on && (bow_bind.flags & MCORB_BOW_MATCH);
    s.undist_job = undist_on;
    s.undist_gen = undist_gen;
    std::fill(s.kps_undist_ok.begin(), s.kps_undist_ok.end(), (uint8_t)0);
    s.h_overflow[0] = 0;
    s.host_results = j.nimg <= kSmallBatch && params.orientation == 0 && !blur_planes &&
                     (!gpu_select || (!j.ext_desc && geom.kcap <= kSelSignalMaxCount));
    s.set_ctl(s.host_results, s.host_results && !gpu_select);
    s.blur_valid = blur_planes;
    return MCORB_OK;
}

int Rig::enqueue_front(Slot &s, int nimg, int *tbl)
{
    const bool ev_on = s.ev_on();
    if (ev_on) HIPCHK(hipEventRecord(s.ev_start, s.st));
    launch_pyramid(s.st, s.d_pyr, geom, d_taps, resize_win, nimg);
    if (ev_on) HIPCHK(hipEventRecord(s.ev_pyr, s.st));
    launch_fast(s.st, s.d_pyr, geom, params.ini_th_fast, params.min_th_fast, d_fasttab + fast_cell_off, s.d_cellkp, s.d_cellcnt, nimg);
    if (ev_on) HIPCHK(hipEventRecord(s.ev_fast, s.st));
    launch_compact(s.st, s.d_cellkp, s.d_cellcnt, geom, d_lut, s.d_sorted, s.h_cand, tbl, s.h_overflow, nimg, compact_one_copy);
    if (ev_on) HIPCHK(hipEventRecord(s.ev_c, s.st));
    return MCORB_OK;
}

int Rig::enqueue_tables_to_host(Slot &s, int nimg, bool by_kernel)
{
    const size_t bytes = (size_t)nimg * s.tbl_ints_per_image * sizeof(int);
    if (!by_kernel) HIPCHK(hipMemcpyAsync(s.h_tbl, s.d_tbl, bytes, hipMemcpyDeviceToHost, s.st_copy));
    else launch_copy_to_host(s.st_copy, s.d_tbl, s.h_tbl, bytes);
    HIPCHK(hipEventRecord(s.ev_tables, s.st_copy));
    return MCORB_OK;
}

int Rig::run_extract_phaseA(Slot &s, const Job &j)
{
    TRY(begin_extract(s, j));
    TRY(enqueue_front(s, j.nimg, s.host_results ? s.h_tbl : s.d_tbl));
    if (s.host_results) {
        HIPCHK(hipEventRecord(s.ev_tables, s.st));
    } else {
        HIPCHK(hipStreamWaitEvent(s.st_copy, s.ev_c, 0));
        TRY(enqueue_tables_to_host(s, j.nimg, copy_kernel));
        if (blur_planes) launch_blur(s.st, s.d_pyr, s.d_blur, geom, j.nimg);
    }
    HIPCHK(hipEventRecord(s.ev_blur, s.st));
    HIPCHK(hipGetLastError());
    return MCORB_OK;
}

mcorb_keypoint Rig::make_keypoint(int level, int xl, int yl, float response, float angle) const
{
    mcorb_keypoint kp;
    kp.x = (float)xl; kp.y = (float)yl;
    kp.size = (float)tab.scaled_patch[level];
    kp.angle = angle;
    kp.response = response;
    kp.octave = level;
    kp.class_id = -1;
    if (level != 0) { kp.x *= tab.scale[level]; kp.y *= tab.scale[level]; }
    return kp;
}

void Rig::read_timing(Slot &s, hipEvent_t blur0)
{
    float a = 0, b = 0, c = 0, t = 0;
    ev_elapsed(&a, s.ev_start, s.ev_fast);
    if (blur0) ev_elapsed(&b, blur0, s.ev_blur);
    ev_elapsed(&c, s.ev_desc0, s.ev_desc1);
    s.timing[T_FRONT] = a * 1000.f;
    s.timing[T_DESC] = (b + c) * 1000.f;
    s.timing[T_BLUR] = b * 1000.f;
    s.timing[T_DESCRIBE] = c * 1000.f;
    ev_elapsed(&t, s.ev_start, s.ev_pyr); s.timing[T_PYR] = t * 1000.f;
    ev_elapsed(&t, s.ev_pyr, s.ev_fast); s.timing[T_FAST] = t * 1000.f;
    ev_elapsed(&t, s.ev_fast, s.ev_c); s.timing[T_COMPACT] = t * 1000.f;
}

int Rig::run_select_and_describe(Slot &s, const Job &j, bool then_match)
{
    HIPCHK(wait_event(s.ev_tables));
    LatProf::mark(2);
    if (s.h_overflow[0]) {
        set_error(kCandOverflowMsg);
        (void)hipStreamSynchronize(s.st);
        return MCORB_E_OVERFLOW;
    }
    const auto t0 = std::chrono::steady_clock::now();
    const int L = geom.nlevels, nimg = j.nimg;
    std::atomic<int> bad{0};
    auto select_level = [&](int m, int level, int w) {
        const int *tb = s.tbl(m);
        const int *lo = tb + kTblLvlOff, *shp = tb + kTblShipped;
        const int *bst = tb + kTblHead;
        const BucketWin *win = reinterpret_cast<const BucketWin *>(tb + tbl_win_off(geom.bucketTotal));
        const int n = lo[level + 1] - lo[level];
        std::vector<uint32_t> &out = s.sel_val[(size_t)m * L + level];
        out.resize((size_t)tab.quota[level] + 64);
        std::vector<int> &idx = scratch[w]->idx;
        idx.resize(out.size());
// ... 290 lines not shown
```

mc-slam_amd/csrc/mcorb_engine.h:

```cpp
#pragma once
#include <hip/hip_runtime.h>
#include <stdint.h>

#include <algorithm>
#include <atomic>
#include <condition_variable>
#include <functional>
#include <memory>
#include <mutex>
#include <string>
#include <thread>
#include <vector>

#include "../../include/mcorb.h"
#include "mcorb_common.h"
#include "mcorb_hip.h"
#include "mcorb_kernels.h"
#include "mcorb_select.h"

namespace mcorb {

const char *get_error();

struct Tables {
    int nlevels = 0;
    float scale[kMaxLevels], inv_scale[kMaxLevels], sigma2[kMaxLevels], inv_sigma2[kMaxLevels];
    int quota[kMaxLevels];
    int scaled_patch[kMaxLevels];
    int umax[16];
};
int compute_tables(const mcorb_params &p, Tables &t);

void build_resize_axis(int ssize, int dsize, bool is_x, std::vector<ResizeTap> &out, int pad_to);

int build_geometry(const mcorb_params &p, const Tables &t, int W, int H, Geom &g, std::vector<ResizeTap> &taps,
                   std::vector<uint16_t> *lut = nullptr);
int resize_windows(const Geom &g, const std::vector<ResizeTap> &taps, int win[2 * kMaxLevels]);

static inline size_t align_up(size_t v, size_t a) { return (v + a - 1) / a * a; }
constexpr unsigned kHostMapped = hipHostMallocMapped | hipHostMallocPortable;
constexpr int kSmallBatch = 8;
int usable_cores();

class WorkerPool {
public:
    explicit WorkerPool(int nthreads);
    ~WorkerPool();
    void parallel_for(int n, const std::function<void(int, int)> &fn, int caller_widx = -1);
    int size() const { return (int)threads_.size(); }

private:
    struct Batch {
        const std::function<void(int, int)> *fn;
        std::atomic<int> next{0};
        int n = 0;
        std::atomic<int> done{0};
        std::atomic<int> refs{0};
        std::mutex m;
        std::condition_variable cv;
    };
    void run(int widx);
    std::vector<std::thread> threads_;
    std::mutex m_;
    std::condition_variable cv_;
    std::vector<Batch *> queue_;
    std::atomic<int> pending_{0};
    bool stop_ = false;
};

struct Job {
    enum Kind { NONE, EXTRACT, MATCH, PROCESS } kind = NONE;
    int nimg = 0, nframes = 0, lap0 = 0, lap1 = 0;
    float dist_thresh = 75.f, ratio = 0.85f;
    const void *ext_desc = nullptr;
    const int32_t *ext_counts = nullptr;
    int ext_total = 0;
    const int32_t *ext_sets = nullptr;
    const int32_t *ext_counts_dev = nullptr;
    hipStream_t after_stream = nullptr;
    const int32_t *ext_pairs = nullptr;
    int ext_npairs = 0;
};

class Rig;

enum Timing { T_FRONT, T_SELECT, T_DESC, T_MATCH, T_PYR, T_FAST, T_COMPACT, T_KNN2, T_BLUR, T_DESCRIBE, T_COUNT };

struct EpipolarGate;
void merge_pair_lists(int ncams, const int *counts, const uint32_t *const *idx1, const uint32_t *const *idx2, const int *np,
                      const EpipolarGate *gate, std::vector<int32_t> &tr, int &mergeable_out);

struct BowFrameOut {
    std::vector<int32_t> tracks, n_rays;
    std::vector<uint32_t> words;
};

struct BowImageOut {
    std::vector<uint32_t> bow_ids, fv_nodes;
    std::vector<double> bow_vals;
    std::vector<int32_t> fv_offsets, fv_feats;
};

struct LfFrameOut {
    std::vector<mcorb_lf_feature> feats;
    std::vector<uint32_t> words_fil;
    std::vector<int32_t> src;
    int intramatch_size = 0, mono_size = 0;
    BowImageOut bow;
};

struct UndistBufs {
    Event ev_u0, ev_u1;
    DevBuf<float2> d_undist;
    HostBuf<float2> h_undist;
    bool bound = false;
    int alloc(size_t npoints);
};

struct BowBufs {
    Event ev_b;
// ... 78 lines not shown
    std::vector<std::vector<uint32_t>> sel_val;
    int npairs_done = 0, nframes_done = 0, nimg_done = 0;
    int nsets_local = 0;
    std::vector<std::vector<uint32_t>> m_idx1, m_idx2;
    std::vector<std::vector<int32_t>> tracks;
    std::vector<int> mergeable;
    std::vector<BowFrameOut> bow;
    std::vector<uint8_t> bow_ok;
    std::vector<BowImageOut> bowvec;
    std::vector<uint8_t> bowvec_ok;
    void invalidate_bow()
    {
        std::fill(bow_ok.begin(), bow_ok.end(), (uint8_t)0);
        std::fill(bowvec_ok.begin(), bowvec_ok.end(), (uint8_t)0);
        std::fill(lf_ok.begin(), lf_ok.end(), (uint8_t)0);
    }
    std::vector<LfFrameOut> lf;
    std::vector<uint8_t> lf_ok;
    float timing[T_COUNT] = {};
    bool undist_job = false;
    unsigned undist_gen = 0;
    bool submitted = false;
    int bow_job = 0;
    bool lf_job = false;
    std::vector<std::vector<mcorb_keypoint>> kps_undist;
    std::vector<uint8_t> kps_undist_ok;
    std::mutex undist_m;
    std::vector<int> match_sets, match_counts;
    bool match_external = false;
    bool host_results = false;
    bool ev_on() const { return !(host_results && capturing); }
    struct Ctrl {
        const int *nsel, *setmap;
        const int2 *pairs;
        const uint32_t *sel;
    } ctl = {};
    void set_ctl(bool host_lists, bool host_sel)
    {
        const CtrlView &sel = host_sel ? hc : dc, &lists = host_lists ? hc : dc;
        ctl = {sel.nsel, lists.setmap, lists.pairs, sel.sel};
    }
    std::thread th;
    std::mutex m;
    std::condition_variable cv;
    Job job;
    bool busy = false, quit = false, inline_job = false;
    int status = MCORB_OK;
    std::string err;
    UndistBufs ubuf;
    BowBufs bbuf;
    LfBufs lbuf;
};

struct EpipolarGate {
    const double *F;
    const mcorb_keypoint *const *kps;
    const float *sigma2;
};

class Rig {
public:
    Rig() = default;
    ~Rig();
    int init(const mcorb_params &p, int ncams, int W, int H, int max_frames, int nslots);

    int upload_u8(int slot, const uint8_t *const *images, int nimg, int stride);
    int upload_staged(int slot, int nimg);
    int upload_f32(int slot, const float *const *images, int nimg, int stride_bytes, int channels);
    int submit(int slot, const Job &job);
    int run_sync(int slot, const Job &job);
    int wait(int slot);

    mcorb_params params;
    Tables tab;
    Geom geom;
    int ncams = 0, W = 0, H = 0, max_frames = 0, max_images = 0, npp = 0 ;
    int ext_cap = 0;
    int device = 0;
    DevBuf<ResizeTap> d_taps;
    DevBuf<uint16_t> d_lut;
    DevBuf<uint32_t> d_fasttab;
    int fast_cell_off = 0;
    SelectParams selp[kMaxLevels];
    int resize_win[2 * kMaxLevels] = {};
    std::vector<std::unique_ptr<Slot>> slots;
    std::unique_ptr<WorkerPool> pool;
    int pool_threads = 0;
    int gpu_job_limit = 0;
    int gpu_jobs_running = 0;
    std::mutex gpu_jobs_m;
    std::condition_variable gpu_jobs_cv;
    void gpu_job_begin();
    void gpu_job_end();
    bool upload_pipelined = true;
    std::atomic<int> graph_every{0};
    int select_deep_cap = 4096;
    bool compact_one_copy = false;
    bool select_prof = false;
    bool gpu_select = false;
    int wait_mode = 0;
    hipError_t wait_event(hipEvent_t ev) const;
    std::vector<std::unique_ptr<SelectScratch>> scratch;

    void merge_tracks(Slot &s, int f, const EpipolarGate *gate, std::vector<int32_t> &tr, int &mergeable_out) const;

    std::vector<UndistCam> undist_cams;
    std::vector<uint8_t> undist_set;
    DevBuf<UndistCam> d_undist_cams;
    bool undist_on = false;
    unsigned undist_gen = 0;
    int set_undistortion(int cam, const double *K, const double *dist, int ncoeffs);
    int undist_records(Slot &s, int m0, int n, std::vector<const mcorb_keypoint *> &out);
    int undist_default(Slot &s, int m0, int n, std::vector<const mcorb_keypoint *> &out);
    int max_pairs() const { return std::max(1, npp * max_frames); }

    std::vector<UndistImageCam> imgud_cams;
    std::vector<uint8_t> imgud_set;
    std::vector<std::vector<int16_t>> imgud_map1;
    std::vector<std::vector<uint16_t>> imgud_map2;
    std::vector<DevBuf<int16_t>> d_imgud_map1;
    std::vector<DevBuf<uint16_t>> d_imgud_map2;
    DevBuf<RemapCam> d_remap_cams;
    bool imgud_on = false;
    int set_image_undistortion(int cam, const double *K, const double *dist, int ncoeffs);
    int enqueue_remap(Slot &s, int nimg);

    struct BowBinding {
        int flags = 0, levelsup = 0, L = 0, weighting = 0, scoring = 0;
        double ratio = 0.85;
        const int *child_start = nullptr, *child_count = nullptr, *child_id = nullptr, *word_id = nullptr;
        const void *child_desc = nullptr;
        const double *weight = nullptr;
    };
    BowBinding bow_bind;
    unsigned bow_gen = 0;
    bool lf_on = false;
    int lf_total_feats = 3000;
    std::vector<mcorb_camera> lf_cams;
    DevBuf<LfCam> d_lfcams;
    unsigned lf_gen = 0;
    int set_lf(const mcorb_camera *cams, int total_feats);
    int set_vocabulary(const BowBinding &b);
    int check_job_shape(const Job &j) const;
    int lock_idle_slots(const char *who, std::vector<std::unique_lock<std::mutex>> &locks);

private:
    bool copy_kernel = false;
    bool blur_planes = false;
    void driver(Slot *s);
    int execute(Slot &s, const Job &j);
    int begin_extract(Slot &s, const Job &j);
    int enqueue_front(Slot &s, int nimg, int *tbl);
    int enqueue_tables_to_host(Slot &s, int nimg, bool by_kernel);
    int enqueue_back(Slot &s, const Job &j, bool then_match, bool gpu_sel);
    void read_timing(Slot &s, hipEvent_t blur0);
    mcorb_keypoint make_keypoint(int level, int xl, int yl, float response, float angle) const;
    int run_extract_phaseA(Slot &s, const Job &j);
    int run_select_and_describe(Slot &s, const Job &j, bool then_match);
    int run_gpu_selected(Slot &s, const Job &j, bool then_match);
    int enqueue_gpu_job(Slot &s, const Job &j, bool then_match);
    int enqueue_undistort(Slot &s, int nimg);
    int enqueue_bow(Slot &s, int nimg);
    int prepare_match(Slot &s, const Job &j);
    int enqueue_match(Slot &s, const Job &j, bool ctrl_on_device);
    int finish_match(Slot &s, const Job &j);
};

// ... 22 lines not shown
```

mc-slam_amd/csrc/mcorb_geometry.cpp:

```cpp
#include <math.h>
#include <string.h>

#include "mcorb_engine.h"

namespace mcorb {

static inline int cv_round_f(float v) { return (int)lrintf(v); }
static inline int cv_round_d(double v) { return (int)lrint(v); }
static inline int cv_floor_f(float v) { int i = (int)v; return i - (i > v); }
static inline int cv_ceil_f(float v) { int i = (int)v; return i + (i < v); }

int compute_tables(const mcorb_params &p, Tables &t)
{
    if (p.nlevels < 1 || p.nlevels > kMaxLevels || p.nfeatures < 1 || !(p.scale_factor > 1.0f)) {
        set_error("bad extractor parameters");
        return MCORB_E_ARG;
    }
    const int L = p.nlevels;
    const double sf = (double)p.scale_factor;
    t.nlevels = L;
    t.scale[0] = 1.0f;
    t.sigma2[0] = 1.0f;
    for (int i = 1; i < L; i++) {
        t.scale[i] = (float)((double)t.scale[i - 1] * sf);
// ... 53 lines not shown
    const ResizeTap last = out.size() > first ? out.back() : ResizeTap{0, 0, 0, 0};
    while ((out.size() - first) % pad_to) out.push_back(last);
}

int build_geometry(const mcorb_params &p, const Tables &t, int W, int H, Geom &g, std::vector<ResizeTap> &taps,
                   std::vector<uint16_t> *lut)
{
    memset(&g, 0, sizeof(g));
    taps.clear();
    if (lut) lut->clear();
    g.nlevels = t.nlevels;
    size_t off = 0;
    int cells = 0, tiles = 0, cellCap = 4, buckets = 0;
    for (int l = 0; l < t.nlevels; l++) {
        LevelGeom &L = g.lv[l];
        const float sc = t.inv_scale[l];
        L.w = cv_round_f((float)W * sc);
        L.h = cv_round_f((float)H * sc);
        L.maxBorderX = L.w - kEdge + 3;
        L.maxBorderY = L.h - kEdge + 3;
        const float width = (float)(L.maxBorderX - kMinBorder);
        const float height = (float)(L.maxBorderY - kMinBorder);
        L.nCols = (int)(width / (float)kCellW);
        L.nRows = (int)(height / (float)kCellW);
        if (L.nCols < 1 || L.nRows < 1) {
            set_error("image too small for the reference's 35-px cell grid at level " + std::to_string(l));
            return MCORB_E_SIZE;
        }
        L.wCell = (int)ceilf(width / L.nCols);
        L.hCell = (int)ceilf(height / L.nRows);
        const SelectParams sp = make_select_params(kMinBorder, L.maxBorderX, kMinBorder, L.maxBorderY, t.quota[l], 1, 1);
        if (sp.nIni < 1) {
            set_error("image too tall: DistributeOctTree would have no root node");
            return MCORB_E_SIZE;
        }
        if (sp.nIni > 16) { set_error("image too wide (more than 16 root nodes)"); return MCORB_E_SIZE; }
        L.nIni = sp.nIni;
        L.hX = sp.hX;
        L.depth = sp.depth;
        L.nBuckets = sp.nIni << (2 * sp.depth);
        L.bucket0 = buckets;
        L.quota = t.quota[l];
        buckets += L.nBuckets + 1;
        if (lut) {
            const int W0 = L.maxBorderX - kMinBorder, H0 = L.maxBorderY - kMinBorder;
            L.lutx = (uint32_t)lut->size();
            L.luty = L.lutx + (uint32_t)W0;
            lut->resize(lut->size() + (size_t)W0 + H0);
            path_code_tables(W0, H0, L.nIni, L.hX, L.depth, lut->data() + L.lutx, lut->data() + L.luty);
            while (lut->size() & 7) lut->push_back(0);
        }
        if (L.w > 4096 || L.h > 4096) { set_error("image larger than 4096 px"); return MCORB_E_SIZE; }
        L.pitch = (int)align_up((size_t)L.w, 64);
        L.off = (uint32_t)off;
        off += align_up((size_t)L.pitch * align_up((size_t)L.h, kBlurTileRows), 256);
        L.cell0 = cells;
        cells += L.nCols * L.nRows;
        L.tilesX = (L.w + kBlurTW - 1) / kBlurTW;
        L.tilesY = (L.h + kBlurTH - 1) / kBlurTH;
        L.tile0 = tiles;
        tiles += L.tilesX * L.tilesY;
        cellCap = std::max(cellCap, ((L.wCell + 1) / 2) * ((L.hCell + 1) / 2));
        if (l > 0) {
            L.xtab = (uint32_t)taps.size();
            build_resize_axis(g.lv[l - 1].w, L.w, true, taps, 4);
            L.ytab = (uint32_t)taps.size();
            build_resize_axis(g.lv[l - 1].h, L.h, false, taps, 4);
        }
    }
    g.cells = cells;
    g.tiles = tiles;
    g.bucketTotal = buckets;
    g.cellCap = (int)align_up((size_t)cellCap, 4);
    g.imgBytes = (uint32_t)(off + 256);
    g.kcap = (int)align_up((size_t)p.nfeatures + 4 * t.nlevels + 48, 64);
    if (g.kcap > 65535) { set_error("nfeatures too large (k-NN index is 16 bits)"); return MCORB_E_ARG; }
    g.candCap = (int)align_up((size_t)g.cells * g.cellCap, 4096);
    g.hostCandCap = p.cand_cap > 0 ? p.cand_cap : (int)align_up(std::max((size_t)65536, (size_t)W * H / 4), 4096);
    if (g.hostCandCap > g.candCap) g.hostCandCap = g.candCap;
    if (g.lv[0].nCols * g.lv[0].nRows * g.cellCap > kPickOrderMask) { set_error("image too large (pick order is 23 bits)"); return MCORB_E_SIZE; }
    return MCORB_OK;
}

int resize_windows(const Geom &g, const std::vector<ResizeTap> &taps, int win[2 * kMaxLevels])
{
    for (int l = 1; l < g.nlevels; l++) {
        const LevelGeom &D = g.lv[l];
        int maxc = 16, maxr = 2;
        for (int bx0 = 0; bx0 < D.w; bx0 += 256) {
            const int bx1 = std::min(bx0 + 255, D.w - 1);
            const int a = taps[D.xtab + bx0].s0 & ~15, b = taps[D.xtab + bx1].s1;
            maxc = std::max(maxc, ((b - a) / 16 + 1) * 16);
        }
        for (int by0 = 0; by0 < D.h; by0 += kResizeTileH) {
            const int by1 = std::min(by0 + kResizeTileH - 1, D.h - 1);
            maxr = std::max(maxr, (int)taps[D.ytab + by1].s1 - (int)taps[D.ytab + by0].s0 + 1);
        }
        win[2 * l] = maxc;
        win[2 * l + 1] = maxr;
        if ((size_t)maxc * maxr > 60000) { set_error("scale factor too large for the resize window"); return MCORB_E_ARG; }
    }
    return MCORB_OK;
}

}
```

mc-slam_amd/csrc/mcorb_kernels.h:

```cpp
#pragma once
#include <hip/hip_runtime.h>
#include <vector>
#include "../../include/mcorb.h"
#include "mcorb_common.h"
#include "mcorb_mapping_new.h"
#include "mcorb_pose.h"
#include "mcorb_sac.h"
#include "mcorb_signal.h"
#include "mcorb_track.h"
#include "mcorb_undistort.h"
#include "mcorb_undistort_image.h"

namespace mcorb {

constexpr int kKnnChunk = 4096;
__host__ __device__ inline int knn_chunk_len(int npairs) { return npairs <= 12 ? 256 : npairs <= 24 ? 512 : npairs <= 48 ? 1024 : kKnnChunk; }
constexpr int kKnnQueriesPerBlock = 256;
inline int knn_qblocks(int kcap) { return (kcap + kKnnQueriesPerBlock - 1) / kKnnQueriesPerBlock; }
inline size_t knn_mlist_stride(int kcap) { return (size_t)knn_qblocks(kcap) * kKnnQueriesPerBlock; }
inline size_t knn_part_entries(int max_pairs, int kcap)
{
    size_t need = 0;
    for (int np : {12, 24, 48, max_pairs}) {
        const int n = np < max_pairs ? np : max_pairs, cl = knn_chunk_len(n);
        const size_t e = (size_t)n * ((kcap + cl - 1) / cl) * kcap;
        need = need > e ? need : e;
    }
    return need;
}
constexpr int kKnnExpandBytes = 128;

struct KnnRow { uint32_t idx, d; };
__host__ __device__ inline int knn_idx0(const KnnRow &r) { return (r.idx & 0xffffu) == 0xffffu ? -1 : (int)(r.idx & 0xffffu); }
__host__ __device__ inline int knn_idx1(const KnnRow &r) { return (r.idx >> 16) == 0xffffu ? -1 : (int)(r.idx >> 16); }
__host__ __device__ inline int knn_d0(const KnnRow &r) { return knn_idx0(r) < 0 ? -1 : (int)(r.d & 0x1ffu); }
__host__ __device__ inline int knn_d1(const KnnRow &r) { return knn_idx1(r) < 0 ? -1 : (int)((r.d >> 9) & 0x1ffu); }
__host__ __device__ inline bool knn_accept(const KnnRow &r) { return (r.d >> 18) & 1u; }

hipError_t upload_umax(const int umax[16]);
void launch_stage_f32(hipStream_t st, const float *src, int w, int h, int pitch_f, int channels, size_t img_stride_f,
                      uint8_t *pyr, const Geom &g, int nimg);
struct RemapCam { const int16_t *map1; const uint16_t *map2; int32_t mode, pad; };
__host__ __device__ inline int remap_map_pitch(int w) { return (w + 3) & ~3; }
void launch_stage_f32_raw(hipStream_t st, const float *src, int w, int h, int pitch_f, int channels, size_t img_stride_f,
                          uint8_t *raw, int nimg);
void launch_remap_u8(hipStream_t st, const uint8_t *raw, uint8_t *pyr, const Geom &g, const RemapCam *cams, int ncams, int nimg);
void launch_pyramid(hipStream_t st, uint8_t *pyr, const Geom &g, const ResizeTap *tabs, const int *win, int nimg);
int fast_cell_table(const Geom &g, std::vector<uint32_t> &tab);
void launch_fast(hipStream_t st, const uint8_t *pyr, const Geom &g, int iniTh, int minTh, const uint32_t *cellRec,
                 uint32_t *cell_kp, int *cell_cnt, int nimg);
void launch_compact(hipStream_t st, const uint32_t *cell_kp, const int *cell_cnt, const Geom &g, const uint16_t *lut,
                    uint32_t *sorted_dev, uint32_t *cand, int *tbl, int *overflow, int nimg, bool one_copy = false);
void launch_blur(hipStream_t st, const uint8_t *pyr, uint8_t *blur, const Geom &g, int nimg);
void launch_describe(hipStream_t st, const uint8_t *pyr, const uint8_t *blur, const Geom &g, const uint32_t *sel,
                     const int *nsel, int orientation, uint8_t *desc, float *angles, int nimg,
                     uint8_t *desc_host = nullptr);
void launch_knn2(hipStream_t st, const uint8_t *desc, const int *counts, const int *setmap, int nsets, const int2 *pairs, int npairs,
                 int kcap, void *expanded, int *lcounts, uint2 *part, float dist_thresh, float ratio, KnnRow *out, uint32_t *mlist,
                 int *mcount, hipEvent_t ev_exp, hipEvent_t ev_mid);

int select_cap(const Geom &g);
bool select_fits(const Geom &g);
hipError_t configure_select(const Geom &g);
hipError_t launch_select(hipStream_t st, const int *tbl, const uint32_t *sorted, const Geom &g, uint32_t *sel_val, int *sel_cnt, int *fallback, int nimg,
                         int deep_cap = 4096, bool prof = false);
void launch_assemble(hipStream_t st, const uint32_t *sel_val, const int *sel_cnt, const Geom &g, const float *scale, int lap0, int lap1,
                     uint32_t *sel, uint8_t *resp, int *nsel, int *mono, int *fallback, int nimg,
                     uint32_t *sel_h = nullptr, uint8_t *resp_h = nullptr, unsigned long long *sig_h = nullptr);
hipError_t sort_selftest(const uint64_t *in_dev, int n, uint64_t *out_dev);

void launch_undistort(hipStream_t st, const uint32_t *sel, const int *nsel, int kcap, int nimg, int ncams, const UndistCam *cams,
                      const float *scale, int nlevels, float2 *out);

void launch_copy_to_host(hipStream_t st, const void *src_dev, void *dst_host_mapped, size_t bytes);

void launch_bow_best2(hipStream_t st, const uint8_t *desc, int img0, int kcap, int ncams, int nframes, const float *yv,
                      const int *slot_of, const int2 *node_range, const int *rg_base, const int *node_feats, const int *nfeat, int4 *out);
void launch_bow_fold(hipStream_t st, const BowRes *res, const int *nsel, int kcap, int nimg, int weighting, int scoring, int *out_dev,
                     int *out_host);
void launch_bow_tables(hipStream_t st, const int *fold, int kcap, int ncams, int nframes, const int *nsel, const uint32_t *sel,
                       const float *scale, int nlevels, const float2 *undist, int *slot_of, int *node_feats, int *nfeat, int *rg_base,
                       float *yv, int2 *node_range);
void launch_bow_descend(hipStream_t st, const uint8_t *desc, int n, const int *child_start, const int *child_count,
                        const void *child_desc, const int *child_id, const int *word_id, const double *weight, int nid_level,
                        BowRes *out);

void launch_lf_tracks(hipStream_t st, const int4 *trk, const LfView *views, int ntr, const LfCam *cams, const uint8_t *desc, int kcap,
                      int ncams, LfTrackOut *out);
void launch_tri_selftest(hipStream_t st, const double *x, const double *P, const int *nv, const int *voff, int n, double *X, int *branch);

void launch_kfdb_score(hipStream_t st, const uint32_t *ids, const double *vals, const int *nbow, int stride, const uint32_t *q_ids,
                       const double *q_vals, const int *q_n, const int *q_sel, const int *q_limit, const int *e_list, int nq,
                       int max_limit, int out_stride, double *raw, int *shared);
void launch_kfdb_best2(hipStream_t st, const uint8_t *desc_a, const int *feats_a, const uint8_t *desc_b, size_t desc_stride,
                       const int *feats_b, size_t feats_stride, const int2 *items, int nitems, const int4 *recs, int4 *out);
void launch_kfdb_gather(hipStream_t st, const uint8_t *desc, const int *src, int n, uint8_t *dst);

constexpr int kLmapCullT = 256;
void launch_lmap_cull(hipStream_t st, const mcorb_lmap_view *view, const double *geom, const int *cand, int n, uint32_t *masks);
void launch_lmap_put(hipStream_t st, const int *lids, int n, const double *pt, const double *normal, const uint8_t *src_desc,
                     const int *rows, double *geom, uint8_t *desc);

constexpr int kMapBlock = 64;
void launch_map_triangulate(hipStream_t st, const MapArgs &a, int nblocks_small, int nblocks_any);
void launch_map_depth(hipStream_t st, const double Rcw[9], const double tcw[3], const double *geom, const int *lids, int n, double *z);
void launch_map_put(hipStream_t st, const MapOut *rec, const int2 *put, int n, double *geom, int32_t *nrays);
void launch_map_gates(hipStream_t st, const MapGateCases &c, int n, MapOut *out);
void launch_map_refine_new(hipStream_t st, const MapNewArgs &n, int nblocks_small, int nblocks_any);
void launch_map_refine_cases(hipStream_t st, const MapRefineCases &c, int n, MapOut *out, MapNewExtra *extra);


void launch_lmap_observe(hipStream_t st, const LmCentres &cen, int ncams, const LmObsItem *items, int n, double *geom, int32_t *nrays);
void launch_lmap_update(hipStream_t st, const LmUpdItem *items, int n, double max_diff, double *geom, LmUpdOut *out);
void launch_lmap_put_rays(hipStream_t st, const int32_t *lids, const int32_t *vals, int n, int32_t *nrays);

constexpr int kTrackProjectT = 256;
void launch_track_project(hipStream_t st, const mcorb_track_view &view, const double *geom, const int *cand, int n, float2 *xy,
                          uint8_t *valid, double *pts);
constexpr int kTrackMatchWaves = 4;
constexpr int kTrackMatchQ = 4;
constexpr int kTrackMatchT = 64 * kTrackMatchWaves;
void launch_track_match(hipStream_t st, const TrFrame &frame, int ncams, const float2 *kp_xy, const uint8_t *kp_desc, const uint8_t *lm_desc,
                        const int *cand, int n, const float2 *xy, const uint8_t *valid, double max_d2, int max_hamming, TrBest *best);
void launch_track_points(hipStream_t st, const uint32_t *sel, const int *nsel, int kcap, int img0, int ncams, const float *scale,
                         int nlevels, float2 *out);
void launch_track_compact(hipStream_t st, int ncams, int n, const uint8_t *valid, const float2 *xy, const TrBest *best, TrRow *rows,
                          int32_t *n_proj);
constexpr int kTrackDedupT = 256;
void launch_track_dedup(hipStream_t st, const TrFrame &frame, int ncams, const float2 *kp_xy, int n, const uint8_t *valid, const TrBest *best,
                        uint32_t *owner, unsigned long long *val, int32_t *slot, uint8_t *win, TrMatch *matches, int32_t *n_match);
// ... 41 lines not shown
```

mc-slam_amd/csrc/mcorb_kernels.hip:

```cpp
#include <hip/hip_runtime.h>
#include <stdint.h>
#include <string.h>
#include <vector>

#include "mcorb_common.h"
#include "mcorb_device.h"
#include "mcorb_kernels.h"

namespace mcorb {

constexpr int kResizeRows = kResizeTileH;

template <int NF>
__global__ __launch_bounds__(256) void k_resize(uint8_t *__restrict__ pyr, Geom g, int level,
                                                const ResizeTap *__restrict__ tabs, int srcPitch, int srcRows)
{
    extern __shared__ __attribute__((aligned(16))) uint8_t win[];
    const LevelGeom &D = g.lv[level];
    const LevelGeom &S = g.lv[level - 1];
    const int img = blockIdx.z;
    uint8_t *base = pyr + (size_t)img * g.imgBytes;
    const int tid = threadIdx.x;
    const int bx0 = blockIdx.x * 256, by0 = blockIdx.y * kResizeRows;
    const int bx1 = min(bx0 + 255, D.w - 1), by1 = min(by0 + kResizeRows - 1, D.h - 1);
    const int sx0 = tabs[D.xtab + bx0].s0 & ~15, sx1 = tabs[D.xtab + bx1].s1;
    const int sy0 = tabs[D.ytab + by0].s0, sy1 = tabs[D.ytab + by1].s1;
    const int nq = ((sx1 - sx0) >> 4) + 1, nr = sy1 - sy0 + 1;
    const int wave = wave_uniform(tid >> 6);
    const int wy0 = by0 + wave * (kResizeRows / 4);
    uint2 ytap;
    {
        const int l = tid & 63;
        const int dy = min(wy0 + (l < kResizeRows / 4 ? l : 0), D.h - 1);
        ytap = *reinterpret_cast<const uint2 *>(tabs + D.ytab + dy);
    }
    const int dx4 = bx0 + (tid & 63) * 4;
    const int dxc = min(dx4, ((D.w + 3) & ~3) - 4);
    const uint4 t01 = *reinterpret_cast<const uint4 *>(tabs + D.xtab + dxc);
    const uint4 t23 = *reinterpret_cast<const uint4 *>(tabs + D.xtab + dxc + 2);
    {
        const uint8_t *sp = base + S.off + (size_t)sy0 * S.pitch + sx0;
        uint4 *w128 = reinterpret_cast<uint4 *>(win);
        const int pq = srcPitch >> 4;
        const float rcp_pq = 1.0f / (float)pq;
        if constexpr (NF > 0) {
            uint4 v[NF];
            bool ok[NF];
#pragma unroll
            for (int k = 0; k < NF; k++) {
                const int i = tid + 256 * k, ic = min(i, nr * pq - 1);
                const int r = (int)(((float)ic + 0.5f) * rcp_pq), q = ic - r * pq;
                ok[k] = i < nr * pq && q < nq;
                v[k] = *reinterpret_cast<const uint4 *>(sp + (size_t)r * S.pitch + 16 * min(q, nq - 1));
            }
            const int spare = (srcPitch >> 4) * srcRows;
#pragma unroll
            for (int k = 0; k < NF; k++) w128[ok[k] ? tid + 256 * k : spare] = v[k];
        } else {
            for (int i = tid; i < nr * pq; i += 256) {
                const int r = (int)(((float)i + 0.5f) * rcp_pq), q = i - r * pq;
                if (q < nq) w128[i] = *reinterpret_cast<const uint4 *>(sp + (size_t)r * S.pitch + 16 * q);
            }
        }
    }
    __syncthreads();
    asm volatile("" ::"v"(ytap.x), "v"(ytap.y), "v"(t01.x), "v"(t01.y), "v"(t01.z), "v"(t01.w), "v"(t23.x), "v"(t23.y), "v"(t23.z), "v"(t23.w));
    if (dx4 >= D.w) return;
    const uint32_t tw[8] = {t01.x, t01.y, t01.z, t01.w, t23.x, t23.y, t23.z, t23.w};
    int s0[4], s1[4], a0[4], a1[4];
#pragma unroll
    for (int k = 0; k < 4; k++) {
        s0[k] = (int)(tw[2 * k] & 0xffff) - sx0;
        s1[k] = (int)(tw[2 * k] >> 16) - sx0;
        a0[k] = (int)(short)(tw[2 * k + 1] & 0xffff);
        a1[k] = (int)(short)(tw[2 * k + 1] >> 16);
    }
    const uint32_t mask = dx4 + 4 > D.w ? 0xffffffffu >> (8 * (dx4 + 4 - D.w)) : 0xffffffffu;
    int rowA = -1, rowB = -1;
    uint32_t HA[4], HB[4];
    const uint32_t ldsWin = (uint32_t)(uintptr_t)(__attribute__((address_space(3))) void *)win;
    uint32_t sb[4];
#pragma unroll
    for (int k = 0; k < 4; k++) sb[k] = ldsWin + (uint32_t)s0[k];
    auto hrow = [&](int sr, uint32_t *Hout) {
        const uint32_t ro = (uint32_t)__mul24(sr - sy0, srcPitch);
        const uint32_t ad0 = sb[0] + ro, ad1 = sb[1] + ro, ad2 = sb[2] + ro, ad3 = sb[3] + ro;
        uint32_t x0, x1, x2, x3, x4, x5, x6, x7;
        asm volatile("ds_read_u8 %0, %8\n\tds_read_u8 %1, %8 offset:1\n\t"
                     "ds_read_u8 %2, %9\n\tds_read_u8 %3, %9 offset:1\n\t"
                     "ds_read_u8 %4, %10\n\tds_read_u8 %5, %10 offset:1\n\t"
                     "ds_read_u8 %6, %11\n\tds_read_u8 %7, %11 offset:1\n\t"
                     "s_waitcnt lgkmcnt(0)"
                     : "=&v"(x0), "=&v"(x1), "=&v"(x2), "=&v"(x3), "=&v"(x4), "=&v"(x5), "=&v"(x6), "=&v"(x7)
                     : "v"(ad0), "v"(ad1), "v"(ad2), "v"(ad3)
                     : "memory");
        Hout[0] = (__umul24(x0, (uint32_t)a0[0]) + __umul24(x1, (uint32_t)a1[0])) >> 4;
        Hout[1] = (__umul24(x2, (uint32_t)a0[1]) + __umul24(x3, (uint32_t)a1[1])) >> 4;
        Hout[2] = (__umul24(x4, (uint32_t)a0[2]) + __umul24(x5, (uint32_t)a1[2])) >> 4;
        Hout[3] = (__umul24(x6, (uint32_t)a0[3]) + __umul24(x7, (uint32_t)a1[3])) >> 4;
    };
#pragma unroll
    for (int rr = 0; rr < kResizeRows / 4; rr++) {
        const int dy = wy0 + rr;
        if (dy >= D.h) break;
        const uint32_t ys = (uint32_t)__builtin_amdgcn_readlane((int)ytap.x, rr), yc = (uint32_t)__builtin_amdgcn_readlane((int)ytap.y, rr);
        const int r0 = (int)(ys & 0xffff), r1 = (int)(ys >> 16);
        if (r0 != rowA) {
            if (r0 == rowB) {
#pragma unroll
                for (int k = 0; k < 4; k++) HA[k] = HB[k];
            } else {
                hrow(r0, HA);
            }
            rowA = r0;
        }
        if (r1 != rowB) {
            if (r1 == rowA) {
#pragma unroll
                for (int k = 0; k < 4; k++) HB[k] = HA[k];
            } else {
                hrow(r1, HB);
            }
            rowB = r1;
        }
        const uint32_t b0 = yc & 0xffff, b1 = yc >> 16;
        uint32_t p0[4], p1[4];
#pragma unroll
        for (int k = 0; k < 4; k++) {
            p0[k] = __umul24(b0, HA[k]) + 0x20000u;
            p1[k] = __umul24(b1, HB[k]);
        }
        uint32_t t01v, t23v;
        asm("v_add_u32_sdwa %0, %1, %2 dst_sel:DWORD dst_unused:UNUSED_PAD src0_sel:WORD_1 src1_sel:WORD_1" : "=v"(t01v) : "v"(p0[0]), "v"(p1[0]));
        asm("v_add_u32_sdwa %0, %1, %2 dst_sel:WORD_1 dst_unused:UNUSED_PRESERVE src0_sel:WORD_1 src1_sel:WORD_1" : "+v"(t01v) : "v"(p0[1]), "v"(p1[1]));
        asm("v_add_u32_sdwa %0, %1, %2 dst_sel:DWORD dst_unused:UNUSED_PAD src0_sel:WORD_1 src1_sel:WORD_1" : "=v"(t23v) : "v"(p0[2]), "v"(p1[2]));
        asm("v_add_u32_sdwa %0, %1, %2 dst_sel:WORD_1 dst_unused:UNUSED_PRESERVE src0_sel:WORD_1 src1_sel:WORD_1" : "+v"(t23v) : "v"(p0[3]), "v"(p1[3]));
        const u16x2 s01 = __builtin_bit_cast(u16x2, t01v) >> (unsigned short)2, s23 = __builtin_bit_cast(u16x2, t23v) >> (unsigned short)2;
        const uint32_t out = __builtin_amdgcn_perm(__builtin_bit_cast(uint32_t, s23), __builtin_bit_cast(uint32_t, s01), 0x06040200u);
        *reinterpret_cast<uint32_t *>(base + D.off + (size_t)dy * D.pitch + dx4) = out & mask;
    }
}


struct FastCell {
    int on;
    int cell;
    int ph;
    int wi, hi;
    int rows;
    int g0, ng;
    int R;
    float rcp_ng;
    uint32_t headMask, tailMask;
    uint32_t org;
    const uint8_t *src;
    int pitch;
};

constexpr int kFastCellRecDw = 8;
__device__ __forceinline__ void fast_cell_setup(const uint8_t *pyr, const Geom &g, int img, int cell, const uint32_t *__restrict__ rec, FastCell &C)
{
    const uint4 r = *reinterpret_cast<const uint4 *>(rec + (size_t)cell * kFastCellRecDw);
    const uint2 r4 = *reinterpret_cast<const uint2 *>(rec + (size_t)cell * kFastCellRecDw + 4);
    C.cell = cell;
    C.src = pyr + (size_t)img * g.imgBytes + r.x;
    C.org = r.y;
    C.pitch = (int)r.z;
    C.rows = (int)(r.w & 0xff);
    C.wi = (int)((r.w >> 8) & 0xff);
    C.hi = (int)((r.w >> 16) & 0xff);
    C.on = (int)((r.w >> 24) & 1);
    C.ph = (int)((r.w >> 25) & 3);
    C.g0 = (int)(r4.x & 0xff);
    C.ng = (int)((r4.x >> 8) & 0xff);
    C.R = (int)(r4.x >> 16);
    C.rcp_ng = __uint_as_float(r4.y);
    const uint2 r6 = *reinterpret_cast<const uint2 *>(rec + (size_t)cell * kFastCellRecDw + 6);
    C.headMask = r6.x;
    C.tailMask = r6.y;
}

int fast_cell_table(const Geom &g, std::vector<uint32_t> &tab)
{
    const int off = (int)tab.size();
    tab.resize(tab.size() + (size_t)g.cells * kFastCellRecDw, 0u);
    for (int level = 0; level < g.nlevels; level++) {
        const LevelGeom &L = g.lv[level];
        for (int cl = 0; cl < L.nCols * L.nRows; cl++) {
            const int ci = cl / L.nCols, cj = cl - ci * L.nCols;
            const int iniY = kMinBorder + ci * L.hCell;
            int maxY = iniY + L.hCell + 6;
            const int iniX = kMinBorder + cj * L.wCell;
            int maxX = iniX + L.wCell + 6;
            const bool skip = (iniY >= L.maxBorderY - 3) || (iniX >= L.maxBorderX - 6);
            if (maxY > L.maxBorderY) maxY = L.maxBorderY;
            if (maxX > L.maxBorderX) maxX = L.maxBorderX;
            const int cols = maxX - iniX, rows = maxY - iniY;
            const int wi = cols - 6, hi = rows - 6;
            const int ph = iniX & 3, g0 = (ph + 3) >> 2;
            const bool on = !(skip || wi <= 0 || hi <= 0);
            const int ng = on ? ((ph + 2 + wi) >> 2) - g0 + 1 : 1;
            uint32_t *r = tab.data() + off + (size_t)(L.cell0 + cl) * kFastCellRecDw;
            r[0] = on ? (uint32_t)(L.off + (size_t)iniY * L.pitch + (iniX - ph)) : 0u;
            r[1] = ((uint32_t)(ci * L.hCell) << 20) + ((uint32_t)(cj * L.wCell - ph) << 8);
            r[2] = (uint32_t)L.pitch;
            r[3] = on ? ((uint32_t)rows | ((uint32_t)wi << 8) | ((uint32_t)hi << 16) | (1u << 24) | ((uint32_t)ph << 25)) : 0u;
            r[4] = (uint32_t)g0 | ((uint32_t)ng << 8) | ((uint32_t)(64 / ng) << 16);
            const float rcp = 1.0f / (float)ng;
            uint32_t bits;
            memcpy(&bits, &rcp, 4);
            r[5] = bits;
            auto pxmask = [&](int G) {
                static const uint32_t bit[4] = {1u << 15, 1u, 1u << 31, 1u << 16};
                uint32_t m = 0;
                for (int j = 0; j < 4; j++) {
                    const int x = 4 * G + j - (ph + 3);
                    if (x >= 0 && x < wi) m |= bit[j];
                }
                return m;
            };
            r[6] = on ? pxmask(g0) : 0u;
            r[7] = on ? pxmask(g0 + ng - 1) : 0u;
// ... 1063 lines not shown
    if (lane == 0) {
#pragma unroll
        for (int u = 0; u < kKnnQT; u++) wcnt[wave * kKnnQT + u] = __popcll(bal[u]);
    }
    __syncthreads();
    int before = 0;
    for (int i = 0; i < wave * kKnnQT; i++) before += wcnt[i];
    uint32_t *ml = mlist + (size_t)pair * (qblocks * kKnnQueriesPerBlock) + qb;
#pragma unroll
    for (int u = 0; u < kKnnQT; u++) {
        if ((bal[u] >> lane) & 1) ml[lane_rank(bal[u], before)] = packed[u];
        before += __popcll(bal[u]);
    }
    if (wave == kKnnWaves - 1 && lane == 0) mcount[pair * qblocks + qbi] = before;
}

__device__ __forceinline__ void knn_insert(uint32_t key, uint32_t &k0, uint32_t &k1)
{
    const uint32_t hi = key > k0 ? key : k0;
    k1 = hi < k1 ? hi : k1;
    k0 = key < k0 ? key : k0;
}

__global__ __launch_bounds__(1024) void k_knn2_finalize(const uint2 *__restrict__ part, const int *__restrict__ counts,
                                                        const int2 *__restrict__ pairs, int kcap, int nchunks, int chunkLen,
                                                        float dist_thresh, float ratio, KnnRow *__restrict__ out,
                                                        uint32_t *__restrict__ mlist, int *__restrict__ mcount, int qblocks)
{
    __shared__ int wsum[16];
    __shared__ int s_run;
    const int pair = blockIdx.x, tid = threadIdx.x, lane = tid & 63, wave = tid >> 6;
    const int2 qt = pairs[pair];
    const int nq = min(max(counts[qt.x], 0), kcap), nt = min(max(counts[qt.y], 0), kcap);
    const int used = (nt + chunkLen - 1) / chunkLen;
    if (tid == 0) s_run = 0;
    __syncthreads();
    for (int base = 0; base < nq; base += 1024) {
        const int q = base + tid;
        uint32_t acc = 0, t0 = 0;
        if (q < nq) {
            uint32_t k0 = 0xffffffffu, k1 = 0xffffffffu;
            for (int c = 0; c < used; c += 4) {
                uint2 p[4];
#pragma unroll
                for (int u = 0; u < 4; u++)
                    p[u] = c + u < used ? part[((size_t)pair * nchunks + c + u) * kcap + q] : uint2{0xffffffffu, 0xffffffffu};
#pragma unroll
                for (int u = 0; u < 4; u++) {
                    knn_insert(p[u].x, k0, k1);
                    knn_insert(p[u].y, k0, k1);
                }
            }
            const bool v0 = k0 != 0xffffffffu, v1 = k1 != 0xffffffffu;
            const uint32_t d0 = v0 ? k0 >> 16 : 0u, d1 = v1 ? k1 >> 16 : 0u;
            if (v0 && v1) {
                const float f0 = (float)d0, f1 = (float)d1;
                acc = (f0 < __fmul_rn(ratio, f1)) && !(f0 > dist_thresh);
            }
            t0 = k0 & 0xffffu;
            KnnRow r;
            r.idx = (v0 ? t0 : 0xffffu) | ((v1 ? (k1 & 0xffffu) : 0xffffu) << 16);
            r.d = d0 | (d1 << 9) | (acc << 18);
            out[(size_t)pair * kcap + q] = r;
        }
        const unsigned long long b = __ballot(acc != 0);
        if (lane == 0) wsum[wave] = __popcll(b);
        __syncthreads();
        int before = s_run;
        for (int w = 0; w < wave; w++) before += wsum[w];
        if (acc) mlist[(size_t)pair * (qblocks * kKnnQueriesPerBlock) + lane_rank(b, before)] = ((uint32_t)q << 16) | t0;
        __syncthreads();
        if (tid == 0) {
            int tot = 0;
            for (int w = 0; w < 16; w++) tot += wsum[w];
            s_run += tot;
        }
        __syncthreads();
    }
    if (tid < qblocks) mcount[pair * qblocks + tid] = tid == 0 ? s_run : 0;
}

hipError_t upload_umax(const int umax[16]) { return hipMemcpyToSymbol(HIP_SYMBOL(c_umax), umax, 16 * sizeof(int)); }

void launch_pyramid(hipStream_t st, uint8_t *pyr, const Geom &g, const ResizeTap *tabs, const int *win, int nimg)
{
    for (int l = 1; l < g.nlevels; l++) {
        dim3 grid((g.lv[l].w + 255) / 256, (g.lv[l].h + kResizeRows - 1) / kResizeRows, nimg);
        const int srcPitch = win[2 * l], srcRows = win[2 * l + 1];
        const int chunks = (srcPitch >> 4) * srcRows, nf = (chunks + 255) / 256;
        const size_t lds = (size_t)srcPitch * srcRows + 16;
        const auto kern = nf <= 4 ? k_resize<4> : nf <= 8 ? k_resize<8> : k_resize<0>;
        hipLaunchKernelGGL(kern, grid, dim3(256), lds, st, pyr, g, l, tabs, srcPitch, srcRows);
    }
}

void fast_layout(const Geom &g, int &tp, int &rows)
{
    int pitch = 0;
    rows = 0;
    for (int l = 0; l < g.nlevels; l++) {
        const int p = ((3 + g.lv[l].wCell + 6 + 15) >> 4) << 4;
        pitch = pitch > p ? pitch : p;
        rows = rows > g.lv[l].hCell + 6 ? rows : g.lv[l].hCell + 6;
    }
    tp = pitch <= 48 ? 48 : (pitch <= 64 ? 64 : 80);
}

void launch_fast(hipStream_t st, const uint8_t *pyr, const Geom &g, int iniTh, int minTh, const uint32_t *cellRec,
                 uint32_t *cell_kp, int *cell_cnt, int nimg)
{
    int tp, rows;
    fast_layout(g, tp, rows);
    const int cap = kFastListCap;
    const int tileB = (rows * tp + 15) & ~15, scB = ((rows - 4) * tp + 15) & ~15;
    const size_t lds = 16 + (size_t)tileB + 16 + (size_t)scB + 16 + (size_t)cap * 2;
    dim3 grid(g.cells, nimg);
    if (iniTh < 1) iniTh = 1;
    if (minTh < 1) minTh = 1;
    if (iniTh > 255) iniTh = 255;
    if (minTh > 255) minTh = 255;
    const auto kern = tp == 48 ? k_fast_cells<48> : tp == 64 ? k_fast_cells<64> : k_fast_cells<80>;
    hipLaunchKernelGGL(kern, grid, dim3(64), lds, st, pyr, g, iniTh, minTh, tileB, scB, cap, cellRec, cell_kp, cell_cnt);
}

void launch_compact(hipStream_t st, const uint32_t *cell_kp, const int *cell_cnt, const Geom &g, const uint16_t *lut,
                    uint32_t *sorted_dev, uint32_t *cand, int *tbl, int *overflow, int nimg, bool one_copy)
{
    int maxb = 1, maxc = 1, maxwh = 2;
    for (int l = 0; l < g.nlevels; l++) {
        maxb = maxb > g.lv[l].nBuckets ? maxb : g.lv[l].nBuckets;
        maxc = maxc > g.lv[l].nCols * g.lv[l].nRows ? maxc : g.lv[l].nCols * g.lv[l].nRows;
        const int wh = (g.lv[l].maxBorderX - kMinBorder) + (g.lv[l].maxBorderY - kMinBorder);
        maxwh = maxwh > wh ? maxwh : wh;
    }
    const int bktCap = (maxb + 1 + 3) & ~3;
    const int wg = nimg <= 8 ? 1024 : 512;
    const int cellsCap = (maxc + 8 + 7) & ~7;
    const size_t ldsTail = (size_t)(cellsCap + maxwh + 8) * sizeof(uint16_t);
    const bool fits = (size_t)(2 * kCompactCopies * bktCap) * sizeof(int) + ldsTail <= 64 * 1024;
    const int copies = fits && !one_copy ? kCompactCopies : 1;
    const size_t lds = (size_t)(2 * copies * bktCap) * sizeof(int) + ldsTail;
    const dim3 grid(nimg, g.nlevels);
    const auto kern = wg == 1024 ? (copies == 1 ? k_compact<1024, 4, 1> : k_compact<1024, 4, kCompactCopies>)
                                 : (copies == 1 ? k_compact<512, 4, 1> : k_compact<512, 4, kCompactCopies>);
    hipLaunchKernelGGL(kern, grid, dim3(wg), lds, st, cell_kp, cell_cnt, g, lut, sorted_dev, cand, tbl, overflow, bktCap, cellsCap);
}

void launch_blur(hipStream_t st, const uint8_t *pyr, uint8_t *blur, const Geom &g, int nimg)
{
    dim3 grid(g.tiles, nimg);
    hipLaunchKernelGGL(k_blur, grid, dim3(256), 0, st, pyr, blur, g);
}

void launch_describe(hipStream_t st, const uint8_t *pyr, const uint8_t *blur, const Geom &g, const uint32_t *sel,
                     const int *nsel, int orientation, uint8_t *desc, float *angles, int nimg, uint8_t *desc_host)
{
    if (orientation) {
        dim3 grid((g.kcap + 3) / 4, nimg);
        hipLaunchKernelGGL(k_describe_oriented, grid, dim3(256), 0, st, pyr, blur, g, sel, nsel, desc, angles);
    } else {
        dim3 grid((g.kcap + 4 * kDescPerWave - 1) / (4 * kDescPerWave), nimg);
        if (blur) hipLaunchKernelGGL(k_describe, grid, dim3(256), 0, st, blur, g, sel, nsel, desc);
        else hipLaunchKernelGGL(k_describe_fused, dim3(grid.x * nimg), dim3(256), 0, st, pyr, g, sel, nsel, desc, (int)grid.x, desc_host);
    }
}

void launch_knn2(hipStream_t st, const uint8_t *desc, const int *counts, const int *setmap, int nsets, const int2 *pairs, int npairs,
                 int kcap, void *expanded, int *lcounts, uint2 *part, float dist_thresh, float ratio, KnnRow *out, uint32_t *mlist,
                 int *mcount, hipEvent_t ev_exp, hipEvent_t ev_mid)
{
    uint4 *E = reinterpret_cast<uint4 *>(expanded);
    hipLaunchKernelGGL(k_expand, dim3((kcap + 255) / 256, nsets), dim3(256), 0, st, desc, counts, setmap, kcap, E, lcounts);
    if (ev_exp) (void)hipEventRecord(ev_exp, st);
    const int chunkLen = knn_chunk_len(npairs), nchunks = (kcap + chunkLen - 1) / chunkLen;
    const int qblocks = knn_qblocks(kcap), units = npairs * nchunks;
// ... 15 lines not shown
```

Baseline: 39600 frames/s.

## Restructure pyramid resize into persistent vertical segments with prefetch and tail bands

Replaces the one-tile-per-block resize with a planned launch. Each workgroup now walks a vertical segment of a 256-pixel strip, prefetching the next source window into LDS while it computes the current one. The segment height is chosen from the CU count to keep enough workgroups per CU, and narrow leftover columns are handled by separate band workgroups instead of mostly idle full strips. Grid order is XCD-aware. The cost is extra kernel complexity, more synchronisation, and host-side plan code, plus new API functions to inspect the plan.

```diff
diff --git a/include/mcorb.h b/include/mcorb.h
--- a/include/mcorb.h
+++ b/include/mcorb.h
@@ -116,6 +116,7 @@
 int mcorb_rig_kcap(mcorb_rig *r);
 int mcorb_rig_host_threads(mcorb_rig *r);
 int mcorb_rig_info(mcorb_rig *r, int32_t out[8]);
+int mcorb_rig_resize_plan(mcorb_rig *r, int level, int nimg, int32_t out[12]);
 void *mcorb_rig_desc_device_ptr(mcorb_rig *r, int slot);
 void *mcorb_rig_stream(mcorb_rig *r, int slot);
 int mcorb_rig_export_descriptors(mcorb_rig *r, int slot, void *dst_dev, int32_t *counts_host, int nimg);
@@ -470,6 +471,7 @@
 int mcorb_host_select(const uint32_t *packed, int n, int minX, int maxX, int minY, int maxY,
                       int nfeatures_level, int wCell, int hCell, int32_t *out_idx, int cap);
 int mcorb_host_resize_axis(int ssize, int dsize, int is_x, int32_t *quads);
+int mcorb_host_resize_plan(int sw, int sh, int dw, int dh, int nimg, int cus, int32_t out[12]);
 int mcorb_host_geometry(const mcorb_params *p, int w, int h, int32_t *six_per_level);
 int mcorb_host_triangulate(const double *x, const double *P, int nv, double X[3]);
 int mcorb_host_triangulate_branch(const double *x, const double *P, int nv, double X[3], int32_t *branch);
diff --git a/mc-slam_amd/__init__.py b/mc-slam_amd/__init__.py
--- a/mc-slam_amd/__init__.py
+++ b/mc-slam_amd/__init__.py
@@ -10,6 +10,8 @@
 TH_HIGH = 100
 TH_LOW = 75
 HISTO_LENGTH = 30
+RESIZE_PLAN_FIELDS = ("pitch", "rows", "strips", "rem", "band_groups", "band_rows", "band_pitch", "band_win_rows", "band_wgs",
+                      "seg_rows", "segments", "cus")
 
 
 def _u8(a):
@@ -352,12 +354,18 @@
         p = buf[:n.value]
         return ((p >> 8) & 0xfff).astype(np.int32), (p >> 20).astype(np.int32), (p & 0xff).astype(np.int32)
 
-    def info(self):
+    def info(self, nimg=None):
         o = np.zeros(8, np.int32)
         _lib.check(self.L.mcorb_rig_info(self.h_rig, o.ctypes.data))
         d = dict(zip(("kcap", "cells", "tiles", "cell_cap", "cand_cap", "bucket_total", "img_bytes", "nlevels"), (int(v) for v in o)))
         d["host_threads"] = int(self.L.mcorb_rig_host_threads(self.h_rig))
+        d["resize"] = [None] + [self.resize_plan(l, nimg or self.ncams * self.max_frames) for l in range(1, d["nlevels"])]
         return d
+
+    def resize_plan(self, level, nimg):
+        o = np.zeros(12, np.int32)
+        _lib.check(self.L.mcorb_rig_resize_plan(self.h_rig, level, nimg, o.ctypes.data))
+        return dict(zip(RESIZE_PLAN_FIELDS, (int(v) for v in o)))
 
     def select_mode(self):
         return {1: "host", 2: "gpu"}[self.L.mcorb_rig_select_mode(self.h_rig)]
diff --git a/mc-slam_amd/_lib.py b/mc-slam_amd/_lib.py
--- a/mc-slam_amd/_lib.py
+++ b/mc-slam_amd/_lib.py
@@ -182,6 +182,7 @@
     "mcorb_rig_kcap": (_i, [_vp]),
     "mcorb_rig_host_threads": (_i, [_vp]),
     "mcorb_rig_info": (_i, [_vp, _vp]),
+    "mcorb_rig_resize_plan": (_i, [_vp, _i, _i, _vp]),
     "mcorb_rig_desc_device_ptr": (_vp, [_vp, _i]),
     "mcorb_rig_stream": (_vp, [_vp, _i]),
     "mcorb_rig_export_descriptors": (_i, [_vp, _i, _vp, _vp, _i]),
@@ -216,6 +217,7 @@
     "mcorb_rig_obtain_lf_features_frames": (_i, [_vp, _i, _i, _i, _vp, _vp, _vp, _vp, _vp, _i, _vp, _i, _vp, _i, _vp, _vp, _vp, _vp, _i, _vp]),
     "mcorb_host_select": (_i, [_vp, _i, _i, _i, _i, _i, _i, _i, _i, _vp, _i]),
     "mcorb_host_resize_axis": (_i, [_i, _i, _i, _vp]),
+    "mcorb_host_resize_plan": (_i, [_i, _i, _i, _i, _i, _i, _vp]),
     "mcorb_host_triangulate": (_i, [_vp, _vp, _i, _vp]),
     "mcorb_host_triangulate_branch": (_i, [_vp, _vp, _i, _vp, _vp]),
     "mcorb_rig_set_lf": (_i, [_vp, _vp, _i]),
diff --git a/mc-slam_amd/csrc/mcorb_api.cpp b/mc-slam_amd/csrc/mcorb_api.cpp
--- a/mc-slam_amd/csrc/mcorb_api.cpp
+++ b/mc-slam_amd/csrc/mcorb_api.cpp
@@ -475,6 +475,12 @@
     const Geom &g = r->rig.geom;
     out[0] = g.kcap; out[1] = g.cells; out[2] = g.tiles; out[3] = g.cellCap; out[4] = g.candCap; out[5] = g.bucketTotal;
     out[6] = (int32_t)g.imgBytes; out[7] = g.nlevels;
+    return MCORB_OK;
+}
+int mcorb_rig_resize_plan(mcorb_rig *r, int level, int nimg, int32_t out[12])
+{
+    if (!r || !out || level < 1 || level >= r->rig.geom.nlevels || nimg < 1) return MCORB_E_ARG;
+    resize_plan_ints(r->rig.resize_plans[level], r->rig.geom.lv[level].h, nimg, r->rig.cus, out);
     return MCORB_OK;
 }
 void *mcorb_rig_desc_device_ptr(mcorb_rig *r, int slot)
diff --git a/mc-slam_amd/csrc/mcorb_api_extractor.cpp b/mc-slam_amd/csrc/mcorb_api_extractor.cpp
--- a/mc-slam_amd/csrc/mcorb_api_extractor.cpp
+++ b/mc-slam_amd/csrc/mcorb_api_extractor.cpp
@@ -272,6 +272,27 @@
     return MCORB_OK;
 }
 
+int mcorb_host_resize_plan(int sw, int sh, int dw, int dh, int nimg, int cus, int32_t out[12])
+{
+    if (sw < 1 || sh < 1 || dw < 1 || dh < 1 || dw > 4096 || dh > 4096 || sw > 65535 || sh > 65535 || nimg < 1 || cus < 1 || !out)
+        return MCORB_E_ARG;
+    Geom g;
+    memset(&g, 0, sizeof(g));
+    g.nlevels = 2;
+    g.lv[0].w = sw; g.lv[0].h = sh;
+    g.lv[1].w = dw; g.lv[1].h = dh;
+    std::vector<ResizeTap> taps;
+    g.lv[1].xtab = 0;
+    build_resize_axis(sw, dw, true, taps, 4);
+    g.lv[1].ytab = (uint32_t)taps.size();
+    build_resize_axis(sh, dh, false, taps, 4);
+    ResizePlan plan[kMaxLevels];
+    const int st = resize_plan(g, taps, plan);
+    if (st != MCORB_OK) return st;
+    resize_plan_ints(plan[1], dh, nimg, cus, out);
+    return MCORB_OK;
+}
+
 int mcorb_host_geometry(const mcorb_params *p, int w, int h, int32_t *six)
 {
     if (!p || !six) return MCORB_E_ARG;
diff --git a/mc-slam_amd/csrc/mcorb_common.h b/mc-slam_amd/csrc/mcorb_common.h
--- a/mc-slam_amd/csrc/mcorb_common.h
+++ b/mc-slam_amd/csrc/mcorb_common.h
@@ -140,4 +140,25 @@
 
 struct ResizeTap { uint16_t s0, s1; int16_t c0, c1; };
 
+struct ResizePlan {
+    int pitch, rows;
+    int strips;
+    int rem;
+    int bandGroups;
+    int bandRows;
+    int bandPitch, bandWinRows;
+    int bandWgs;
+};
+constexpr int kResizeWgsPerCu = 32;
+#if defined(__HIPCC__)
+__host__ __device__
+#endif
+inline int resize_segment_rows(int h, int strips, int nimg, int cus)
+{
+    int seg = (h + kResizeTileH - 1) / kResizeTileH * kResizeTileH;
+    while (seg > kResizeTileH && (long long)strips * ((h + seg - 1) / seg) * nimg < (long long)kResizeWgsPerCu * cus)
+        seg = (seg / 2 + kResizeTileH - 1) / kResizeTileH * kResizeTileH;
+    return seg;
 }
+
+}
diff --git a/mc-slam_amd/csrc/mcorb_engine.cpp b/mc-slam_amd/csrc/mcorb_engine.cpp
--- a/mc-slam_amd/csrc/mcorb_engine.cpp
+++ b/mc-slam_amd/csrc/mcorb_engine.cpp
@@ -70,7 +70,8 @@
         selp[l] = make_select_params(kMinBorder, geom.lv[l].maxBorderX, kMinBorder, geom.lv[l].maxBorderY, tab.quota[l],
                                      geom.lv[l].wCell, geom.lv[l].hCell);
     if (taps.empty()) taps.push_back(ResizeTap{0, 0, 0, 0});
-    TRY(resize_windows(geom, taps, resize_win));
+    TRY(resize_plan(geom, taps, resize_plans));
+    cus = prop.multiProcessorCount;
     TRY(d_taps.alloc(taps.size()));
     HIPCHK(hipMemcpy(d_taps, taps.data(), taps.size() * sizeof(ResizeTap), hipMemcpyHostToDevice));
     TRY(d_lut.alloc(lut.size() + 8));
@@ -355,7 +356,7 @@
 {
     const bool ev_on = s.ev_on();
     if (ev_on) HIPCHK(hipEventRecord(s.ev_start, s.st));
-    launch_pyramid(s.st, s.d_pyr, geom, d_taps, resize_win, nimg);
+    launch_pyramid(s.st, s.d_pyr, geom, d_taps, resize_plans, cus, nimg);
     if (ev_on) HIPCHK(hipEventRecord(s.ev_pyr, s.st));
     launch_fast(s.st, s.d_pyr, geom, params.ini_th_fast, params.min_th_fast, d_fasttab + fast_cell_off, s.d_cellkp, s.d_cellcnt, nimg);
     if (ev_on) HIPCHK(hipEventRecord(s.ev_fast, s.st));
diff --git a/mc-slam_amd/csrc/mcorb_engine.h b/mc-slam_amd/csrc/mcorb_engine.h
--- a/mc-slam_amd/csrc/mcorb_engine.h
+++ b/mc-slam_amd/csrc/mcorb_engine.h
@@ -35,7 +35,8 @@
 
 int build_geometry(const mcorb_params &p, const Tables &t, int W, int H, Geom &g, std::vector<ResizeTap> &taps,
                    std::vector<uint16_t> *lut = nullptr);
-int resize_windows(const Geom &g, const std::vector<ResizeTap> &taps, int win[2 * kMaxLevels]);
+int resize_plan(const Geom &g, const std::vector<ResizeTap> &taps, ResizePlan plan[kMaxLevels]);
+void resize_plan_ints(const ResizePlan &P, int h, int nimg, int cus, int32_t out[12]);
 
 static inline size_t align_up(size_t v, size_t a) { return (v + a - 1) / a * a; }
 constexpr unsigned kHostMapped = hipHostMallocMapped | hipHostMallocPortable;
@@ -280,7 +281,8 @@
     DevBuf<uint32_t> d_fasttab;
     int fast_cell_off = 0;
     SelectParams selp[kMaxLevels];
-    int resize_win[2 * kMaxLevels] = {};
+    ResizePlan resize_plans[kMaxLevels] = {};
+    int cus = 0;
     std::vector<std::unique_ptr<Slot>> slots;
     std::unique_ptr<WorkerPool> pool;
     int pool_threads = 0;
diff --git a/mc-slam_amd/csrc/mcorb_geometry.cpp b/mc-slam_amd/csrc/mcorb_geometry.cpp
--- a/mc-slam_amd/csrc/mcorb_geometry.cpp
+++ b/mc-slam_amd/csrc/mcorb_geometry.cpp
@@ -159,25 +159,63 @@
     return MCORB_OK;
 }
 
-int resize_windows(const Geom &g, const std::vector<ResizeTap> &taps, int win[2 * kMaxLevels])
-{
+int resize_plan(const Geom &g, const std::vector<ResizeTap> &taps, ResizePlan plan[kMaxLevels])
+{
+    constexpr int kBandWindowBytes = 20480;
     for (int l = 1; l < g.nlevels; l++) {
         const LevelGeom &D = g.lv[l];
+        ResizePlan &P = plan[l];
+        P = ResizePlan{};
+        const ResizeTap *xt = taps.data() + D.xtab, *yt = taps.data() + D.ytab;
+        const int groups = (D.w + 3) / 4, full = groups / 64;
+        P.rem = groups % 64;
+        P.strips = full + (P.rem > 32 ? 1 : 0);
         int maxc = 16, maxr = 2;
-        for (int bx0 = 0; bx0 < D.w; bx0 += 256) {
-            const int bx1 = std::min(bx0 + 255, D.w - 1);
-            const int a = taps[D.xtab + bx0].s0 & ~15, b = taps[D.xtab + bx1].s1;
+        for (int s = 0; s < P.strips; s++) {
+            const int bx0 = 256 * s, bx1 = std::min(bx0 + 255, D.w - 1);
+            const int a = xt[bx0].s0 & ~15, b = xt[bx1].s1;
             maxc = std::max(maxc, ((b - a) / 16 + 1) * 16);
         }
         for (int by0 = 0; by0 < D.h; by0 += kResizeTileH) {
             const int by1 = std::min(by0 + kResizeTileH - 1, D.h - 1);
-            maxr = std::max(maxr, (int)taps[D.ytab + by1].s1 - (int)taps[D.ytab + by0].s0 + 1);
-        }
-        win[2 * l] = maxc;
-        win[2 * l + 1] = maxr;
+            maxr = std::max(maxr, (int)yt[by1].s1 - (int)yt[by0].s0 + 1);
+        }
+        P.pitch = maxc;
+        P.rows = maxr;
         if ((size_t)maxc * maxr > 60000) { set_error("scale factor too large for the resize window"); return MCORB_E_ARG; }
+        if (P.rem >= 1 && P.rem <= 32) {
+            int rp = 1;
+            while (rp < P.rem) rp *= 2;
+            P.bandGroups = rp;
+            const int bands = 4 * (64 / rp);
+            const int a = xt[256 * full].s0 & ~15, b = xt[D.w - 1].s1;
+            P.bandPitch = ((b - a) / 16 + 1) * 16;
+            auto window_rows = [&](int rows_per_wg) {
+                int r = 1;
+                for (int by0 = 0; by0 < D.h; by0 += rows_per_wg) {
+                    const int by1 = std::min(by0 + rows_per_wg - 1, D.h - 1);
+                    r = std::max(r, (int)yt[by1].s1 - (int)yt[by0].s0 + 1);
+                }
+                return r;
+            };
+            int rb = 8;
+            while (rb > 1 && bands * (rb / 2) >= D.h) rb /= 2;
+            while (rb > 1 && (size_t)P.bandPitch * window_rows(bands * rb) > kBandWindowBytes) rb /= 2;
+            P.bandRows = rb;
+            P.bandWinRows = window_rows(bands * rb);
+            P.bandWgs = (D.h + bands * rb - 1) / (bands * rb);
+            if ((size_t)P.bandPitch * P.bandWinRows > 60000) { set_error("scale factor too large for the resize window"); return MCORB_E_ARG; }
+        }
     }
     return MCORB_OK;
 }
 
-}
+void resize_plan_ints(const ResizePlan &P, int h, int nimg, int cus, int32_t out[12])
+{
+    const int seg = resize_segment_rows(h, P.strips, nimg, cus);
+    const int32_t v[12] = {P.pitch, P.rows, P.strips, P.rem, P.bandGroups, P.bandRows, P.bandPitch, P.bandWinRows, P.bandWgs,
+                           seg, (h + seg - 1) / seg, cus};
+    memcpy(out, v, sizeof(v));
+}
+
+}
diff --git a/mc-slam_amd/csrc/mcorb_kernels.h b/mc-slam_amd/csrc/mcorb_kernels.h
--- a/mc-slam_amd/csrc/mcorb_kernels.h
+++ b/mc-slam_amd/csrc/mcorb_kernels.h
@@ -45,7 +45,7 @@
 void launch_stage_f32_raw(hipStream_t st, const float *src, int w, int h, int pitch_f, int channels, size_t img_stride_f,
                           uint8_t *raw, int nimg);
 void launch_remap_u8(hipStream_t st, const uint8_t *raw, uint8_t *pyr, const Geom &g, const RemapCam *cams, int ncams, int nimg);
-void launch_pyramid(hipStream_t st, uint8_t *pyr, const Geom &g, const ResizeTap *tabs, const int *win, int nimg);
+void launch_pyramid(hipStream_t st, uint8_t *pyr, const Geom &g, const ResizeTap *tabs, const ResizePlan *plan, int cus, int nimg);
 int fast_cell_table(const Geom &g, std::vector<uint32_t> &tab);
 void launch_fast(hipStream_t st, const uint8_t *pyr, const Geom &g, int iniTh, int minTh, const uint32_t *cellRec,
                  uint32_t *cell_kp, int *cell_cnt, int nimg);
diff --git a/mc-slam_amd/csrc/mcorb_kernels.hip b/mc-slam_amd/csrc/mcorb_kernels.hip
--- a/mc-slam_amd/csrc/mcorb_kernels.hip
+++ b/mc-slam_amd/csrc/mcorb_kernels.hip
@@ -1,6 +1,7 @@
 #include <hip/hip_runtime.h>
 #include <stdint.h>
 #include <string.h>
+#include <algorithm>
 #include <vector>
 
 #include "mcorb_common.h"
@@ -10,134 +11,285 @@
 namespace mcorb {
 
 constexpr int kResizeRows = kResizeTileH;
-
-template <int NF>
-__global__ __launch_bounds__(256) void k_resize(uint8_t *__restrict__ pyr, Geom g, int level,
-                                                const ResizeTap *__restrict__ tabs, int srcPitch, int srcRows)
-{
-    extern __shared__ __attribute__((aligned(16))) uint8_t win[];
-    const LevelGeom &D = g.lv[level];
-    const LevelGeom &S = g.lv[level - 1];
-    const int img = blockIdx.z;
-    uint8_t *base = pyr + (size_t)img * g.imgBytes;
-    const int tid = threadIdx.x;
-    const int bx0 = blockIdx.x * 256, by0 = blockIdx.y * kResizeRows;
-    const int bx1 = min(bx0 + 255, D.w - 1), by1 = min(by0 + kResizeRows - 1, D.h - 1);
-    const int sx0 = tabs[D.xtab + bx0].s0 & ~15, sx1 = tabs[D.xtab + bx1].s1;
+constexpr bool kResizePrefetch = true;
+constexpr bool kResizeXcdOrder = true;
+constexpr bool kResizeTwoWindows = false;
+
+struct ResizeCols {
+    uint32_t sb[4];
+    uint32_t a0[4], a1[4];
+    uint32_t mask;
+};
+__device__ __forceinline__ ResizeCols resize_cols(const uint4 &t01, const uint4 &t23, int sx0, uint32_t ldsWin, int dx4, int w)
+{
+    const uint32_t tw[8] = {t01.x, t01.y, t01.z, t01.w, t23.x, t23.y, t23.z, t23.w};
+    ResizeCols c;
+#pragma unroll
+    for (int k = 0; k < 4; k++) {
+        c.sb[k] = ldsWin + (uint32_t)((int)(tw[2 * k] & 0xffff) - sx0);
+        c.a0[k] = (uint32_t)(int)(short)(tw[2 * k + 1] & 0xffff);
+        c.a1[k] = (uint32_t)(int)(short)(tw[2 * k + 1] >> 16);
+    }
+    c.mask = dx4 + 4 > w ? (dx4 < w ? 0xffffffffu >> (8 * (dx4 + 4 - w)) : 0u) : 0xffffffffu;
+    return c;
+}
+__device__ __forceinline__ void resize_hrow(const ResizeCols &c, uint32_t ro, uint32_t *Hout)
+{
+    const uint32_t ad0 = c.sb[0] + ro, ad1 = c.sb[1] + ro, ad2 = c.sb[2] + ro, ad3 = c.sb[3] + ro;
+    uint32_t x0, x1, x2, x3, x4, x5, x6, x7;
+    asm volatile("ds_read_u8 %0, %8\n\tds_read_u8 %1, %8 offset:1\n\t"
+                 "ds_read_u8 %2, %9\n\tds_read_u8 %3, %9 offset:1\n\t"
+                 "ds_read_u8 %4, %10\n\tds_read_u8 %5, %10 offset:1\n\t"
+                 "ds_read_u8 %6, %11\n\tds_read_u8 %7, %11 offset:1\n\t"
+                 "s_waitcnt lgkmcnt(0)"
+                 : "=&v"(x0), "=&v"(x1), "=&v"(x2), "=&v"(x3), "=&v"(x4), "=&v"(x5), "=&v"(x6), "=&v"(x7)
+                 : "v"(ad0), "v"(ad1), "v"(ad2), "v"(ad3)
+                 : "memory");
+    Hout[0] = (__umul24(x0, c.a0[0]) + __umul24(x1, c.a1[0])) >> 4;
+    Hout[1] = (__umul24(x2, c.a0[1]) + __umul24(x3, c.a1[1])) >> 4;
+    Hout[2] = (__umul24(x4, c.a0[2]) + __umul24(x5, c.a1[2])) >> 4;
+    Hout[3] = (__umul24(x6, c.a0[3]) + __umul24(x7, c.a1[3])) >> 4;
+}
+__device__ __forceinline__ uint32_t resize_vert(uint32_t b0, uint32_t b1, const uint32_t *HA, const uint32_t *HB)
+{
+    uint32_t p0[4], p1[4];
+#pragma unroll
+    for (int k = 0; k < 4; k++) {
+        p0[k] = __umul24(b0, HA[k]) + 0x20000u;
+        p1[k] = __umul24(b1, HB[k]);
+    }
+    uint32_t t01v, t23v;
+    asm("v_add_u32_sdwa %0, %1, %2 dst_sel:DWORD dst_unused:UNUSED_PAD src0_sel:WORD_1 src1_sel:WORD_1" : "=v"(t01v) : "v"(p0[0]), "v"(p1[0]));
+    asm("v_add_u32_sdwa %0, %1, %2 dst_sel:WORD_1 dst_unused:UNUSED_PRESERVE src0_sel:WORD_1 src1_sel:WORD_1" : "+v"(t01v) : "v"(p0[1]), "v"(p1[1]));
+    asm("v_add_u32_sdwa %0, %1, %2 dst_sel:DWORD dst_unused:UNUSED_PAD src0_sel:WORD_1 src1_sel:WORD_1" : "=v"(t23v) : "v"(p0[2]), "v"(p1[2]));
+    asm("v_add_u32_sdwa %0, %1, %2 dst_sel:WORD_1 dst_unused:UNUSED_PRESERVE src0_sel:WORD_1 src1_sel:WORD_1" : "+v"(t23v) : "v"(p0[3]), "v"(p1[3]));
+    const u16x2 s01 = __builtin_bit_cast(u16x2, t01v) >> (unsigned short)2, s23 = __builtin_bit_cast(u16x2, t23v) >> (unsigned short)2;
+    return __builtin_amdgcn_perm(__builtin_bit_cast(uint32_t, s23), __builtin_bit_cast(uint32_t, s01), 0x06040200u);
+}
+
+__device__ __forceinline__ void resize_bands(uint8_t *__restrict__ base, const LevelGeom &D, const LevelGeom &S,
+                                             const ResizeTap *__restrict__ tabs, const ResizePlan &P, int k, uint8_t *win)
+{
+    const int tid = threadIdx.x, lane = tid & 63, wave = tid >> 6;
+    const int lg = __ffs(P.bandGroups) - 1, bands = 64 >> lg, rb = P.bandRows;
+    const int rowsWg = 4 * bands * rb;
+    const int by0 = k * rowsWg, by1 = min(by0 + rowsWg, D.h) - 1;
+    const int dx0 = (((D.w + 3) >> 2) & ~63) * 4;
+    const int sx0 = tabs[D.xtab + dx0].s0 & ~15, sx1 = tabs[D.xtab + D.w - 1].s1;
     const int sy0 = tabs[D.ytab + by0].s0, sy1 = tabs[D.ytab + by1].s1;
     const int nq = ((sx1 - sx0) >> 4) + 1, nr = sy1 - sy0 + 1;
-    const int wave = wave_uniform(tid >> 6);
-    const int wy0 = by0 + wave * (kResizeRows / 4);
-    uint2 ytap;
-    {
-        const int l = tid & 63;
-        const int dy = min(wy0 + (l < kResizeRows / 4 ? l : 0), D.h - 1);
-        ytap = *reinterpret_cast<const uint2 *>(tabs + D.ytab + dy);
-    }
-    const int dx4 = bx0 + (tid & 63) * 4;
+    const int row0 = by0 + (wave * bands + (lane >> lg)) * rb;
+    const int dx4 = dx0 + (lane & (P.bandGroups - 1)) * 4;
     const int dxc = min(dx4, ((D.w + 3) & ~3) - 4);
     const uint4 t01 = *reinterpret_cast<const uint4 *>(tabs + D.xtab + dxc);
     const uint4 t23 = *reinterpret_cast<const uint4 *>(tabs + D.xtab + dxc + 2);
     {
         const uint8_t *sp = base + S.off + (size_t)sy0 * S.pitch + sx0;
         uint4 *w128 = reinterpret_cast<uint4 *>(win);
-        const int pq = srcPitch >> 4;
+        const int pq = P.bandPitch >> 4;
         const float rcp_pq = 1.0f / (float)pq;
-        if constexpr (NF > 0) {
-            uint4 v[NF];
-            bool ok[NF];
-#pragma unroll
-            for (int k = 0; k < NF; k++) {
-                const int i = tid + 256 * k, ic = min(i, nr * pq - 1);
+        for (int i0 = 0; i0 < nr * pq; i0 += 1024) {
+            uint4 v[4];
+#pragma unroll
+            for (int u = 0; u < 4; u++) {
+                const int ic = min(i0 + tid + 256 * u, nr * pq - 1);
                 const int r = (int)(((float)ic + 0.5f) * rcp_pq), q = ic - r * pq;
-                ok[k] = i < nr * pq && q < nq;
-                v[k] = *reinterpret_cast<const uint4 *>(sp + (size_t)r * S.pitch + 16 * min(q, nq - 1));
-            }
-            const int spare = (srcPitch >> 4) * srcRows;
-#pragma unroll
-            for (int k = 0; k < NF; k++) w128[ok[k] ? tid + 256 * k : spare] = v[k];
+                v[u] = *reinterpret_cast<const uint4 *>(sp + (size_t)r * S.pitch + 16 * min(q, nq - 1));
+            }
+#pragma unroll
+            for (int u = 0; u < 4; u++) {
+                const int i = i0 + tid + 256 * u;
+                w128[i < nr * pq ? i : pq * P.bandWinRows] = v[u];
+            }
+        }
+    }
+    __syncthreads();
+    if (dx4 >= D.w) return;
+    uint2 ytap[8];
+#pragma unroll
+    for (int rr = 0; rr < 8; rr++)
+        if (rr < rb) ytap[rr] = *reinterpret_cast<const uint2 *>(tabs + D.ytab + min(row0 + rr, D.h - 1));
+    const uint32_t ldsWin = (uint32_t)(uintptr_t)(__attribute__((address_space(3))) void *)win;
+    const ResizeCols c = resize_cols(t01, t23, sx0, ldsWin, dx4, D.w);
+    uint8_t *const dcol = base + D.off + dx4;
+    const int dPitch = D.pitch;
+#pragma unroll
+    for (int rr = 0; rr < 8; rr++) {
+        if (rr >= rb) break;
+        const int dy = row0 + rr;
+        const uint32_t ys = ytap[rr].x, yc = ytap[rr].y;
+        uint32_t HA[4], HB[4];
+        resize_hrow(c, (uint32_t)__mul24((int)(ys & 0xffff) - sy0, P.bandPitch), HA);
+        resize_hrow(c, (uint32_t)__mul24((int)(ys >> 16) - sy0, P.bandPitch), HB);
+        const uint32_t out = resize_vert(yc & 0xffff, yc >> 16, HA, HB);
+        if (dy < D.h) *reinterpret_cast<uint32_t *>(dcol + (uint32_t)__mul24(dy, dPitch)) = out & c.mask;
+    }
+}
+
+template <int NF>
+__global__ __launch_bounds__(256) void k_resize(uint8_t *__restrict__ pyr, Geom g, int level, const ResizeTap *__restrict__ tabs,
+                                                ResizePlan P, int segH, int nseg)
+{
+    extern __shared__ __attribute__((aligned(16))) uint8_t win[];
+    const LevelGeom &D = g.lv[level];
+    const LevelGeom &S = g.lv[level - 1];
+    const int wgsPerImg = (int)gridDim.x;
+    const int wgLaunch = (int)(blockIdx.y * gridDim.x + blockIdx.x);
+    const int wg = kResizeXcdOrder ? xcd_remap(wgLaunch, wgsPerImg * (int)gridDim.y) : wgLaunch;
+    const int img = wg / wgsPerImg, bx = wg - img * wgsPerImg;
+    uint8_t *base = pyr + (size_t)img * g.imgBytes;
+    const int tid = threadIdx.x;
+    if (bx >= P.strips * nseg) {
+        resize_bands(base, D, S, tabs, P, bx - P.strips * nseg, win);
+        return;
+    }
+    const int seg = bx / P.strips, strip = bx - seg * P.strips;
+    const int bx0 = strip * 256, bx1 = min(bx0 + 255, D.w - 1);
+    const int y0 = seg * segH, yEnd = min(y0 + segH, D.h);
+    const int nsteps = (yEnd - y0 + kResizeRows - 1) / kResizeRows;
+    const int lane = tid & 63, wave = wave_uniform(tid >> 6);
+    const int tapRow = lane == 8 ? 0 : lane == 9 ? kResizeRows - 1 : wave * (kResizeRows / 4) + (lane < 8 ? lane : 0);
+    auto fetch_taps = [&](int t) {
+        return *reinterpret_cast<const uint2 *>(tabs + D.ytab + min(y0 + t * kResizeRows + tapRow, yEnd - 1));
+    };
+    uint2 ytap = fetch_taps(0), ytapN = fetch_taps(1);
+    const int sx0 = tabs[D.xtab + bx0].s0 & ~15, sx1 = tabs[D.xtab + bx1].s1;
+    const int nq = ((sx1 - sx0) >> 4) + 1;
+    const int dx4 = bx0 + lane * 4;
+    const int dxc = min(dx4, ((D.w + 3) & ~3) - 4);
+    const uint4 t01 = *reinterpret_cast<const uint4 *>(tabs + D.xtab + dxc);
+    const uint4 t23 = *reinterpret_cast<const uint4 *>(tabs + D.xtab + dxc + 2);
+    constexpr int NV = NF > 0 ? NF : 1;
+    const int pq = P.pitch >> 4;
+    const float rcp_pq = 1.0f / (float)pq;
+    const uint8_t *sp = base + S.off + sx0;
+    v4i *w128 = reinterpret_cast<v4i *>(win);
+    constexpr bool kPre = kResizePrefetch && NF > 0, kTwo = kResizeTwoWindows && kPre;
+    const int spare = pq * P.rows * (kTwo ? 2 : 1);
+    int fr[NV], fo[NV];
+    v4i v[NV] = {};
+    if constexpr (kPre) {
+#pragma unroll
+        for (int k = 0; k < NF; k++) {
+            const int i = tid + 256 * k;
+            const int r = (int)(((float)i + 0.5f) * rcp_pq), q = i - r * pq;
+            fr[k] = r;
+            fo[k] = q < nq ? 16 * q : -1 - 16 * (nq - 1);
+        }
+    }
+    auto win_load = [&](int sy0, int nr) {
+#pragma unroll
+        for (int k = 0; k < NV; k++) {
+            const int r = sy0 + min(fr[k], nr - 1), o = fo[k] < 0 ? -1 - fo[k] : fo[k];
+            v[k] = *reinterpret_cast<const v4i *>(sp + (uint32_t)(__mul24(r, S.pitch) + o));
+        }
+    };
+    auto win_store = [&](int nr, int buf) {
+#pragma unroll
+        for (int k = 0; k < NV; k++) w128[fr[k] < nr && fo[k] >= 0 ? buf + tid + 256 * k : spare] = v[k];
+    };
+    auto win_stage = [&](int sy0, int nr) {
+        bool ok[NV];
+#pragma unroll
+        for (int k = 0; k < NV; k++) {
+            const int i = tid + 256 * k;
+            const int r = (int)(((float)i + 0.5f) * rcp_pq), q = i - r * pq;
+            ok[k] = r < nr && q < nq;
+            v[k] = *reinterpret_cast<const v4i *>(sp + (uint32_t)(__mul24(sy0 + min(r, nr - 1), S.pitch) + 16 * min(q, nq - 1)));
+        }
+#pragma unroll
+        for (int k = 0; k < NV; k++) w128[ok[k] ? tid + 256 * k : spare] = v[k];
+    };
+    auto win_fill = [&](int sy0, int nr) {
+        const uint8_t *s = sp + (size_t)sy0 * S.pitch;
+        for (int i = tid; i < nr * pq; i += 256) {
+            const int r = (int)(((float)i + 0.5f) * rcp_pq), q = i - r * pq;
+            if (q < nq) w128[i] = *reinterpret_cast<const v4i *>(s + (size_t)r * S.pitch + 16 * q);
+        }
+    };
+    int sy0 = __builtin_amdgcn_readlane((int)ytap.x, 8) & 0xffff;
+    int nr = (int)((uint32_t)__builtin_amdgcn_readlane((int)ytap.x, 9) >> 16) - sy0 + 1;
+    if constexpr (kPre) {
+        win_load(sy0, nr);
+        win_store(nr, 0);
+        __syncthreads();
+    }
+    const uint32_t ldsWin = (uint32_t)(uintptr_t)(__attribute__((address_space(3))) void *)win;
+    const ResizeCols c = resize_cols(t01, t23, sx0, ldsWin, dx4, D.w);
+    const bool inRow = dx4 < D.w;
+    uint8_t *const dcol = base + D.off + dx4;
+    const int dPitch = D.pitch;
+    for (int t = 0; t < nsteps; t++) {
+        const uint2 ytapNN = fetch_taps(kPre ? t + 2 : t + 1);
+        asm volatile("" ::"v"(ytap.x), "v"(ytap.y));
+        if constexpr (kPre) asm volatile("" ::"v"(ytapN.x), "v"(ytapN.y));
+        const int sy0N = __builtin_amdgcn_readlane((int)ytapN.x, 8) & 0xffff;
+        const int nrN = t + 1 < nsteps ? (int)((uint32_t)__builtin_amdgcn_readlane((int)ytapN.x, 9) >> 16) - sy0N + 1 : 0;
+        const int cur = kTwo ? (t & 1) * pq * P.rows : 0;
+        if constexpr (kPre) {
+            if (nrN > 0) win_load(sy0N, nrN);
         } else {
-            for (int i = tid; i < nr * pq; i += 256) {
-                const int r = (int)(((float)i + 0.5f) * rcp_pq), q = i - r * pq;
-                if (q < nq) w128[i] = *reinterpret_cast<const uint4 *>(sp + (size_t)r * S.pitch + 16 * q);
-            }
-        }
-    }
-    __syncthreads();
-    asm volatile("" ::"v"(ytap.x), "v"(ytap.y), "v"(t01.x), "v"(t01.y), "v"(t01.z), "v"(t01.w), "v"(t23.x), "v"(t23.y), "v"(t23.z), "v"(t23.w));
-    if (dx4 >= D.w) return;
-    const uint32_t tw[8] = {t01.x, t01.y, t01.z, t01.w, t23.x, t23.y, t23.z, t23.w};
-    int s0[4], s1[4], a0[4], a1[4];
-#pragma unroll
-    for (int k = 0; k < 4; k++) {
-        s0[k] = (int)(tw[2 * k] & 0xffff) - sx0;
-        s1[k] = (int)(tw[2 * k] >> 16) - sx0;
-        a0[k] = (int)(short)(tw[2 * k + 1] & 0xffff);
-        a1[k] = (int)(short)(tw[2 * k + 1] >> 16);
-    }
-    const uint32_t mask = dx4 + 4 > D.w ? 0xffffffffu >> (8 * (dx4 + 4 - D.w)) : 0xffffffffu;
-    int rowA = -1, rowB = -1;
-    uint32_t HA[4], HB[4];
-    const uint32_t ldsWin = (uint32_t)(uintptr_t)(__attribute__((address_space(3))) void *)win;
-    uint32_t sb[4];
-#pragma unroll
-    for (int k = 0; k < 4; k++) sb[k] = ldsWin + (uint32_t)s0[k];
-    auto hrow = [&](int sr, uint32_t *Hout) {
-        const uint32_t ro = (uint32_t)__mul24(sr - sy0, srcPitch);
-        const uint32_t ad0 = sb[0] + ro, ad1 = sb[1] + ro, ad2 = sb[2] + ro, ad3 = sb[3] + ro;
-        uint32_t x0, x1, x2, x3, x4, x5, x6, x7;
-        asm volatile("ds_read_u8 %0, %8\n\tds_read_u8 %1, %8 offset:1\n\t"
-                     "ds_read_u8 %2, %9\n\tds_read_u8 %3, %9 offset:1\n\t"
-                     "ds_read_u8 %4, %10\n\tds_read_u8 %5, %10 offset:1\n\t"
-                     "ds_read_u8 %6, %11\n\tds_read_u8 %7, %11 offset:1\n\t"
-                     "s_waitcnt lgkmcnt(0)"
-                     : "=&v"(x0), "=&v"(x1), "=&v"(x2), "=&v"(x3), "=&v"(x4), "=&v"(x5), "=&v"(x6), "=&v"(x7)
-                     : "v"(ad0), "v"(ad1), "v"(ad2), "v"(ad3)
-                     : "memory");
-        Hout[0] = (__umul24(x0, (uint32_t)a0[0]) + __umul24(x1, (uint32_t)a1[0])) >> 4;
-        Hout[1] = (__umul24(x2, (uint32_t)a0[1]) + __umul24(x3, (uint32_t)a1[1])) >> 4;
-        Hout[2] = (__umul24(x4, (uint32_t)a0[2]) + __umul24(x5, (uint32_t)a1[2])) >> 4;
-        Hout[3] = (__umul24(x6, (uint32_t)a0[3]) + __umul24(x7, (uint32_t)a1[3])) >> 4;
-    };
-#pragma unroll
-    for (int rr = 0; rr < kResizeRows / 4; rr++) {
-        const int dy = wy0 + rr;
-        if (dy >= D.h) break;
-        const uint32_t ys = (uint32_t)__builtin_amdgcn_readlane((int)ytap.x, rr), yc = (uint32_t)__builtin_amdgcn_readlane((int)ytap.y, rr);
-        const int r0 = (int)(ys & 0xffff), r1 = (int)(ys >> 16);
-        if (r0 != rowA) {
-            if (r0 == rowB) {
-#pragma unroll
-                for (int k = 0; k < 4; k++) HA[k] = HB[k];
+            if (t > 0) __syncthreads();
+            if constexpr (NF > 0) {
+                win_stage(sy0, nr);
             } else {
-                hrow(r0, HA);
-            }
-            rowA = r0;
-        }
-        if (r1 != rowB) {
-            if (r1 == rowA) {
-#pragma unroll
-                for (int k = 0; k < 4; k++) HB[k] = HA[k];
+                win_fill(sy0, nr);
+            }
+            __syncthreads();
+        }
+        if (inRow) {
+            const int wy0 = y0 + t * kResizeRows + wave * (kResizeRows / 4);
+            const uint32_t winOff = (uint32_t)cur * 16u;
+            int rowA = -1, rowB = -1;
+            uint32_t HA[4], HB[4];
+#pragma unroll
+            for (int rr = 0; rr < kResizeRows / 4; rr++) {
+                const int dy = wy0 + rr;
+                if (dy >= yEnd) break;
+                const uint32_t ys = (uint32_t)__builtin_amdgcn_readlane((int)ytap.x, rr), yc = (uint32_t)__builtin_amdgcn_readlane((int)ytap.y, rr);
+                const int r0 = (int)(ys & 0xffff), r1 = (int)(ys >> 16);
+                if (r0 != rowA) {
+                    if (r0 == rowB) {
+#pragma unroll
+                        for (int k = 0; k < 4; k++) HA[k] = HB[k];
+                    } else {
+                        resize_hrow(c, winOff + (uint32_t)__mul24(r0 - sy0, P.pitch), HA);
+                    }
+                    rowA = r0;
+                }
+                if (r1 != rowB) {
+                    if (r1 == rowA) {
+#pragma unroll
+                        for (int k = 0; k < 4; k++) HB[k] = HA[k];
+                    } else {
+                        resize_hrow(c, winOff + (uint32_t)__mul24(r1 - sy0, P.pitch), HB);
+                    }
+                    rowB = r1;
+                }
+                const uint32_t out = resize_vert(yc & 0xffff, yc >> 16, HA, HB);
+                *reinterpret_cast<uint32_t *>(dcol + (uint32_t)__mul24(dy, dPitch)) = out & c.mask;
+            }
+        }
+        if constexpr (kPre) {
+            if (kTwo) {
+                win_store(nrN, pq * P.rows - cur);
+                __syncthreads();
             } else {
-                hrow(r1, HB);
-            }
-            rowB = r1;
-        }
-        const uint32_t b0 = yc & 0xffff, b1 = yc >> 16;
-        uint32_t p0[4], p1[4];
-#pragma unroll
-        for (int k = 0; k < 4; k++) {
-            p0[k] = __umul24(b0, HA[k]) + 0x20000u;
-            p1[k] = __umul24(b1, HB[k]);
-        }
-        uint32_t t01v, t23v;
-        asm("v_add_u32_sdwa %0, %1, %2 dst_sel:DWORD dst_unused:UNUSED_PAD src0_sel:WORD_1 src1_sel:WORD_1" : "=v"(t01v) : "v"(p0[0]), "v"(p1[0]));
-        asm("v_add_u32_sdwa %0, %1, %2 dst_sel:WORD_1 dst_unused:UNUSED_PRESERVE src0_sel:WORD_1 src1_sel:WORD_1" : "+v"(t01v) : "v"(p0[1]), "v"(p1[1]));
-        asm("v_add_u32_sdwa %0, %1, %2 dst_sel:DWORD dst_unused:UNUSED_PAD src0_sel:WORD_1 src1_sel:WORD_1" : "=v"(t23v) : "v"(p0[2]), "v"(p1[2]));
-        asm("v_add_u32_sdwa %0, %1, %2 dst_sel:WORD_1 dst_unused:UNUSED_PRESERVE src0_sel:WORD_1 src1_sel:WORD_1" : "+v"(t23v) : "v"(p0[3]), "v"(p1[3]));
-        const u16x2 s01 = __builtin_bit_cast(u16x2, t01v) >> (unsigned short)2, s23 = __builtin_bit_cast(u16x2, t23v) >> (unsigned short)2;
-        const uint32_t out = __builtin_amdgcn_perm(__builtin_bit_cast(uint32_t, s23), __builtin_bit_cast(uint32_t, s01), 0x06040200u);
-        *reinterpret_cast<uint32_t *>(base + D.off + (size_t)dy * D.pitch + dx4) = out & mask;
+                __syncthreads();
+                win_store(nrN, 0);
+                __syncthreads();
+            }
+        }
+        if constexpr (kPre) {
+            ytap = ytapN;
+            ytapN = ytapNN;
+            sy0 = sy0N;
+            nr = nrN;
+        } else {
+            ytap = ytapNN;
+            sy0 = __builtin_amdgcn_readlane((int)ytap.x, 8) & 0xffff;
+            nr = (int)((uint32_t)__builtin_amdgcn_readlane((int)ytap.x, 9) >> 16) - sy0 + 1;
+        }
     }
 }
 
@@ -1367,15 +1519,16 @@
 
 hipError_t upload_umax(const int umax[16]) { return hipMemcpyToSymbol(HIP_SYMBOL(c_umax), umax, 16 * sizeof(int)); }
 
-void launch_pyramid(hipStream_t st, uint8_t *pyr, const Geom &g, const ResizeTap *tabs, const int *win, int nimg)
+void launch_pyramid(hipStream_t st, uint8_t *pyr, const Geom &g, const ResizeTap *tabs, const ResizePlan *plan, int cus, int nimg)
 {
     for (int l = 1; l < g.nlevels; l++) {
-        dim3 grid((g.lv[l].w + 255) / 256, (g.lv[l].h + kResizeRows - 1) / kResizeRows, nimg);
-        const int srcPitch = win[2 * l], srcRows = win[2 * l + 1];
-        const int chunks = (srcPitch >> 4) * srcRows, nf = (chunks + 255) / 256;
-        const size_t lds = (size_t)srcPitch * srcRows + 16;
+        const ResizePlan &P = plan[l];
+        const int segH = resize_segment_rows(g.lv[l].h, P.strips, nimg, cus), nseg = (g.lv[l].h + segH - 1) / segH;
+        dim3 grid(P.strips * nseg + P.bandWgs, nimg);
+        const int chunks = (P.pitch >> 4) * P.rows, nf = (chunks + 255) / 256;
+        const size_t lds = std::max((size_t)P.pitch * P.rows * (kResizePrefetch && kResizeTwoWindows && nf <= 8 ? 2 : 1), (size_t)P.bandPitch * P.bandWinRows) + 16;
         const auto kern = nf <= 4 ? k_resize<4> : nf <= 8 ? k_resize<8> : k_resize<0>;
-        hipLaunchKernelGGL(kern, grid, dim3(256), lds, st, pyr, g, l, tabs, srcPitch, srcRows);
+        hipLaunchKernelGGL(kern, grid, dim3(256), lds, st, pyr, g, l, tabs, P, segH, nseg);
     }
 }
 
```

Result: no change. 39680 frames/s, median of 4 (+0.2%).
